# tmdt-buw/VQ-VAE-Transformer-Arc-Welding

Hardware: AMD Instinct MI355X
Metric: welding windows/sec (train) VQ-VAE+8-blk Transformer at 1/2/4/8 MI355X (higher is better)
Workload: dtype bf16; 1 GPU; VQ-VAE-Patch reconstruction train step (configs[1]); global_batch=1024, per_gpu_batch=1024, seq_len=200, codebook=512x64, hidden=512, n_resblocks=8, patch=25, parallelism=dp1, optimizer=RAdam(lr 1e-3), operands=bf16 (opt-in), fp32 accumulation and master weights

## Files before the change

### include/arcweld_amd.h

```cpp
#ifndef ARCWELD_AMD_H
#define ARCWELD_AMD_H

#include <stdint.h>

#ifdef __cplusplus
extern "C" {
#endif

enum { AW_OK = 0, AW_ERR_ARG = -1, AW_ERR_LAUNCH = -2 };
enum { AW_F32 = 0, AW_BF16 = 1 };
enum { AW_ACT_GELU_ERF = 0, AW_ACT_GELU_TANH = 1, AW_ACT_DERIV = 2 };

const char* aw_last_error(void);
int aw_version(void);

typedef struct {
  int M, N, K;
  int a_dtype;
  const void* A; int64_t lda; int a_trans;
  const void* B; int64_t ldb; int b_trans;
  int conv_cin, conv_seg, conv_dir, conv_operand;
  float alpha, beta;
  const float* bias;
  int act;
  const float* pre; int64_t ld_pre;
  const float* resid; int64_t ld_resid;
  float drop_p; uint64_t drop_seed;
  void* C; int64_t ldc; int c_dtype;
  void* C2; int64_t ldc2; int c2_mode; int c2_dtype;
  float drop2_p; uint64_t drop2_seed;
  double* colstats; int stats_mod;
  float* a_rowsum;
  int bias_mod;
  int accumulate, col_mod, col_mul, col_off;
  const uint64_t* seed_ptr;
  int pre_dtype;
  int store_policy;
  int resid_dtype;
} aw_gemm_args;
#define AW_STORE_NT 0
#define AW_STORE_WT 1

int aw_gemm(const aw_gemm_args* args, void* stream);
int64_t aw_gemm_workspace(const aw_gemm_args* args);
int aw_gemm_ws(const aw_gemm_args* args, float* ws, int64_t ws_elems, void* stream);
#define AW_GEMM_MAX_GROUPS 16
int aw_gemm_grouped(const aw_gemm_args* args, int n, void* stream);
int aw_gemm_set_tile(int bm);
int aw_gemm_describe(const aw_gemm_args* args, int* layout, uint32_t* epi, int* tile_rows, int* specialised,
                     int* ragged, int* splits);
int aw_gemm_set_wgrad_policy(int mode);
#define AW_WGRAD_BATCH_MAX 32
int64_t aw_wgrad_batch_workspace(const aw_gemm_args* args, int n);
int aw_wgrad_batch(const aw_gemm_args* args, int n, void* ws, int64_t ws_bytes, void* stream);
int aw_wgrad_set_spin_limit(int polls);

#define AW_RES_CHAIN_MAX 16
#define AW_RES_TAIL_MAX 8
typedef struct {
  int64_t N;
  int H, R;
  int taps, seg;
  const void* a0;
  const void* x0;
  const void* w1[AW_RES_CHAIN_MAX];
  const void* w2[AW_RES_CHAIN_MAX];
  const float* b1[AW_RES_CHAIN_MAX];
  const float* b2[AW_RES_CHAIN_MAX];
  void* dgelu_h[AW_RES_CHAIN_MAX];
  void* a1[AW_RES_CHAIN_MAX];
  void* dgelu_x[AW_RES_CHAIN_MAX];
  void* a[AW_RES_CHAIN_MAX];
  float drop_p;
  uint64_t drop_seed[AW_RES_CHAIN_MAX];
  const uint64_t* seed_ptr;
  int store_policy;
  uint64_t* drop_masks;
  int tail_k1;
  const void* tail_w[AW_RES_TAIL_MAX];
  const float* tail_bias;
  void* tail_y;
  double* tail_colstats;
} aw_res_chain_fwd_args;
typedef struct {
  int64_t N;
  int H, R;
  int taps, seg;
  const void* gx;
  const void* gxo;
  const void* x0;
  const void* w1t[AW_RES_CHAIN_MAX];
  const void* w2t[AW_RES_CHAIN_MAX];
  const void* dgelu_h[AW_RES_CHAIN_MAX];
  const void* dgelu_x[AW_RES_CHAIN_MAX];
  void* gh[AW_RES_CHAIN_MAX];
  void* gxo_out[AW_RES_CHAIN_MAX];
  float drop_p;
  int store_policy;
  const uint64_t* drop_masks;
} aw_res_chain_bwd_args;
int aw_res_chain_fwd(const aw_res_chain_fwd_args* args, void* stream);
int aw_res_chain_bwd(const aw_res_chain_bwd_args* args, void* stream);
int64_t aw_res_dropout_masks_bytes(int64_t N, int R);
int aw_res_dropout_masks(int64_t N, int R, float drop_p, const uint64_t* drop_seed, const uint64_t* seed_ptr,
                         void* masks, void* stream);
#define AW_RES_PACK_MAX 32
int aw_res_pack_weights(const void* const* src, void* const* fwd, void* const* bwd, int n, int taps, void* stream);
int aw_res_pack_weights_mixed(const void* const* src, void* const* fwd, void* const* bwd, const int* job_taps, int n,
                              int taps, void* stream);

int aw_vq_forward(const float* z, const float* E, int64_t N, int K, int D,
                  float* zq, int64_t* idx, float* counts, double* sqerr, void* stream);
int aw_vq_forward_ex(const float* z, const float* E, int64_t N, int K, int D, float* zq, int64_t* idx, float* counts,
                     double* sqerr, void* zq_copy, int copy_dtype, void* stream);
#define AW_VQ_COUNT_GROUPS_MAX 64
int aw_vq_forward_ex2(const float* z, const float* E, int64_t N, int K, int D, float* zq, int64_t* idx, float* counts,
                      int count_groups, double* sqerr, void* zq_copy, int copy_dtype, void* stream);
int aw_vq_finalize(const float* counts, const double* sqerr, int64_t N, int K, int D, float beta,
                   float* loss, float* perplexity, void* stream);
int aw_vq_finalize_ex(const float* counts, int count_groups, const double* sqerr, int64_t N, int K, int D, float beta,
                      float* loss, float* perplexity, void* stream);
int aw_vq_backward(const float* z, const float* E, const int64_t* idx, const float* g_zq, const float* g_loss,
                   int64_t N, int K, int D, float beta, float* dz, float* dE, void* stream);
int aw_vq_backward_ex(const float* z, const float* E, const int64_t* idx, const float* g_zq, const float* g_loss,
                      int64_t N, int K, int D, float beta, float* dz, float* dE, void* dz_copy, int copy_dtype,
                      void* stream);
int aw_vq_cluster_sums(const float* z, const int64_t* idx, int64_t N, int K, int D, float* sums, void* stream);
int aw_kmeans_update(float* means, const float* sums, const float* counts, int K, int D, float* avg, void* stream);
int aw_rvq_ema_update(float* embed, float* embed_avg, float* cluster_size, const float* counts, const float* sums,
                      const float* z, int64_t N, int K, int D, float decay, float eps, float threshold, uint64_t salt,
                      const uint64_t* seed_ptr, float* ws, void* stream);
int aw_rvq_residual(const float* r, const float* zq, int64_t n, float* out, int first, float* r_next, void* stream);
int aw_rvq_backward(const float* res, const float* q, const float* g_zq, const float* g_loss, int nq, int64_t N,
                    int D, float commitment, float* dz, void* stream);

int aw_vq_onehot(const int64_t* idx, int64_t N, int K, float* onehot, void* stream);
int aw_vq_gather(const float* E, const int64_t* idx, int64_t N, int D, float* out, void* stream);

int aw_patchify(const float* x, int64_t B, int L, int C, int P, void* patches, int64_t ldp, int dtype,
                void* stream);
int aw_weight_relayout(const float* W, int O, int I, int k, int tap, int mode, void* out, int64_t ldo,
                       int dtype, void* stream);
#define AW_RELAYOUT_MAX_JOBS 40
typedef struct {
  const float* W;
  void* out;
  int O, I, k, tap, mode;
  int64_t ldo;
} aw_relayout_job;
int aw_weight_relayout_batch(const aw_relayout_job* jobs, int n, int dtype, void* stream);
int aw_weight_grad_scatter(const float* g, int O, int I, int k, int tap, int mode, int64_t ldg, float* G,
                           void* stream);
int aw_cast(const float* in, int64_t n, void* out, int dtype, void* stream);

int aw_unpatch_head_fwd(const float* y, int64_t R, int H, int Q, const float* stats, const float* w2,
                        const float* b2, float* x_hat, void* stream);
int aw_bn_finalize(const double* colstats, int64_t n, int H, const float* gamma, const float* beta,
                   float* running_mean, float* running_var, int64_t* nbt, float eps, float momentum,
                   int training, float* stats, void* stream);
int aw_unpatch_head_bwd1(const float* y, int64_t R, int H, int Q, const float* stats, const float* w2,
                         const float* g_xhat, double* gsums, float* gw2, float* gb2, float* ggamma, float* gbeta,
                         void* stream);
int aw_unpatch_head_bwd2(const float* y, int64_t R, int H, int Q, const float* stats, const float* w2,
                         const float* g_xhat, const double* gsums, int training, void* g_y, int gy_dtype, float* db_y,
                         void* stream);
int aw_unpatch_head_fwd_ex(const void* y, int y_dtype, int64_t R, int H, int Q, const float* stats, const float* w2,
                           const float* b2, float* x_hat, void* stream);
int aw_unpatch_head_bwd1_ex(const void* y, int y_dtype, int64_t R, int H, int Q, const float* stats, const float* w2,
                            const float* g_xhat, double* gsums, float* gw2, float* gb2, float* ggamma, float* gbeta,
                            void* stream);
int aw_unpatch_head_bwd2_ex(const void* y, int y_dtype, int64_t R, int H, int Q, const float* stats, const float* w2,
                            const float* g_xhat, const double* gsums, int training, void* g_y, int gy_dtype,
                            float* db_y, void* stream);
int aw_unpatch_head_fwd_bwd1(const void* y, int y_dtype, int64_t R, int H, int Q, const float* stats, const float* w2,
                             const float* b2, const float* x, const float* gscale, float* x_hat, float* g_xhat,
                             double* sqerr, double* gsums, float* gw2, float* gb2, float* ggamma, float* gbeta,
                             void* stream);
int aw_bn_group_stats(const float* h, int64_t N, int H, int G, double* sums, void* stream);
int aw_bn_group_finalize(const double* sums, int64_t n, int H, int G, const float* gamma, const float* beta,
                         float* running_mean, float* running_var, int64_t* nbt, float eps, float momentum,
                         int training, float* stats, void* stream);
int aw_bn_apply(const float* h, int64_t N, int H, int G, const float* stats, int mode, const float* resid,
                float drop_p, uint64_t drop_seed, const uint64_t* seed_ptr, float* out, void* op, int op_dtype,
                void* stream);
int aw_bn_bwd_reduce(const float* h, int64_t N, int H, int G, const float* stats, const float* g_in, float drop_p,
                     uint64_t drop_seed, const uint64_t* seed_ptr, double* sums, void* stream);
int aw_bn_bwd_apply(const float* h, int64_t N, int H, int G, const float* stats, const float* g_in, float drop_p,
                    uint64_t drop_seed, const uint64_t* seed_ptr, const double* sums, int64_t n, int training,
                    void* dh, int dh_dtype, float* dgamma, float* dbeta, void* stream);
int aw_mse_fwd(const float* a, const float* b, int64_t n, double* sqerr, void* stream);
int aw_mse_bwd(const float* a, const float* b, int64_t n, const float* g, float* ga, void* stream);

int aw_scalar_add(const float* a, const float* b, float* out, void* stream);
int aw_mse_finalize(const double* sqerr, int64_t numel, float* out, void* stream);
int aw_mse_finalize_add(const double* sqerr, int64_t numel, const float* addend, float* out, float* sum, void* stream);

int aw_radam_step(float* param, float* grad, float* exp_avg, float* exp_avg_sq, const int64_t* seg_off,
                  const int64_t* seg_len, const float* seg_wd, const int* seg_active, int nseg, int64_t total, int64_t step,
                  float lr, float beta1, float beta2, float eps, const float* gscale, const int64_t* step_ptr,
                  int zero_grad, void* stream);
#define AW_OPS_PER_SEG 2
typedef struct {
  void* out;
  int O, I, k, tap, mode, dtype;
  int64_t ldo;
} aw_operand_desc;
int aw_radam_step_ops(float* param, float* grad, float* exp_avg, float* exp_avg_sq, const int64_t* seg_off,
                      const int64_t* seg_len, const float* seg_wd, const int* seg_active, int nseg, int64_t total,
                      int64_t step, float lr, float beta1, float beta2, float eps, const float* gscale,
                      const int64_t* step_ptr, const aw_operand_desc* ops, int zero_grad, void* stream);
int aw_counter_add(int64_t* counter, int64_t v, void* stream);
int aw_counter_add_snapshot(int64_t* counter, int64_t v, int64_t* snapshot, void* stream);
int aw_counter_add_snapshot_zero(int64_t* counter, int64_t v, int64_t* snapshot, double* zero, int64_t nzero,
                                 void* stream);
#define AW_NORM_WS 1024
int aw_grad_norm_clip(const float* grad, const int64_t* seg_off, const int64_t* seg_len, const int* seg_active,
                      int nseg, int64_t total, float max_norm, double* ws, float* out_norm, float* out_coef,
                      void* stream);
int aw_scale(float* x, int64_t n, const float* s, void* stream);

int aw_layernorm_fwd(const float* x, int64_t R, int D, const float* w, const float* b, float eps, void* y,
                     int y_dtype, float* mean, float* rstd, void* stream);
int aw_layernorm_bwd(const float* x, const float* dy, int64_t R, int D, const float* w, const float* mean,
                     const float* rstd, float* dx, int accumulate, float* dw, float* db, void* dx2, int dx2_dtype,
                     float drop_p, uint64_t drop_seed, const uint64_t* seed_ptr, void* stream);
int aw_class_head_fwd(const float* xf, int64_t B, int T, int D, const float* w1, const float* b1, const float* W2,
                      const float* b2, float* s, float* out, void* stream);
int aw_class_head_bwd(const float* xf, const float* s, const float* dout, int64_t B, int T, int D, const float* w1,
                      const float* W2, float* dxf, float* dw1, float* db1, float* dW2, float* db2, void* stream);
int aw_embed_fwd(const int64_t* ids, int64_t B, int T, int D, const float* wtok, const float* pe, float* x,
                 void* stream);
int aw_embed_ln_fwd(const int64_t* ids, int64_t B, int T, int D, const float* wtok, const float* pe, float* x,
                    const float* w, const float* b, float eps, void* y, int y_dtype, float* mean, float* rstd,
                    void* stream);
int aw_embed_bwd(const int64_t* ids, int64_t B, int T, int D, const float* dx, float* dwtok, void* stream);
int aw_embed_bwd_sorted(const int64_t* ids, int64_t B, int T, int D, int V, const float* dx, float* dwtok, int* work,
                        void* stream);
int aw_embed_sort(const int64_t* ids, int64_t R, int V, int* work, void* stream);
int aw_embed_bwd_segsum(const int* work, int V, int D, const float* dx, float* dwtok, void* stream);
int aw_attn_fwd(const void* qkv, int64_t B, int T, int n_head, int d, int dtype, void* y, float* lse,
                void* stream);
int aw_attn_bwd(const void* qkv, const void* y, const void* dy, const float* lse, int64_t B, int T, int n_head,
                int d, int dtype, void* dqkv, float* ws, void* stream);
int aw_attn_fwd_dropout(const void* qkv, int64_t B, int T, int n_head, int d, int dtype, void* y, float* lse,
                        float drop_p, uint64_t drop_seed, const uint64_t* seed_ptr, void* stream);
int aw_attn_bwd_dropout(const void* qkv, const void* y, const void* dy, const float* lse, int64_t B, int T,
                        int n_head, int d, int dtype, void* dqkv, float* ws, float drop_p, uint64_t drop_seed,
                        const uint64_t* seed_ptr, void* stream);
int aw_attn_decode(const void* qkv_new, int64_t B, int n_new, int pos0, int n_head, int d, int dtype,
                   void* kv_cache, int Tmax, void* y, void* stream);
int aw_ce_fwd(const float* logits, int64_t R, int V, int64_t ldl, const int64_t* y, int ignore_index,
              double* loss_sum, double* count, float* lse, void* stream);
int aw_ce_bwd(const float* logits, int64_t R, int V, int64_t ldl, const int64_t* y, int ignore_index,
              const float* lse, const double* count, const float* g, void* dlogits, int64_t ldd, int dtype,
              void* stream);
int aw_ce_finalize(const double* loss_sum, const double* count, float* out, void* stream);

int aw_gru_pack_weights(const float* w_hh, int H, int op_dtype, void* w_fwd, void* w_bwd, void* stream);
int aw_gru_step_fwd(int B, int H, int op_dtype, const void* h_prev_op, const float* h_prev, const void* w_fwd,
                    const float* gi, const float* b_hh, float* h, void* h_op, float* saved, void* stream);
int aw_gru_step_bwd(int B, int H, int op_dtype, const void* dgh_next_op, const float* dh_next,
                    const float* saved_next, const void* w_bwd, const float* dy, const float* saved,
                    const float* h_prev, float* dh, float* dgi, float* dgh, void* dgi_op, void* dgh_op, void* stream);
int aw_gru_bias_grad(const float* dg, int64_t rows, int H, float* db, void* stream);

#ifdef __cplusplus
}
#endif
#endif
```

### vq-vae-transformer-arc-welding_amd/arcweld/_native.py

```python
from __future__ import annotations

import ctypes
import os

import torch

PKG_DIR = os.path.dirname(os.path.dirname(os.path.abspath(__file__)))
LIB_PATH = os.environ.get("ARCWELD_LIB") or os.path.join(PKG_DIR, "lib", "libarcweld_amd.so")
HEADER = os.path.join(os.path.dirname(PKG_DIR), "include", "arcweld_amd.h")

AW_F32, AW_BF16 = 0, 1
AW_ACT_GELU_ERF, AW_ACT_GELU_TANH, AW_ACT_DERIV = 0, 1, 2
AW_STORE_NT, AW_STORE_WT = 0, 1

c_i64 = ctypes.c_int64
c_int = ctypes.c_int
c_f = ctypes.c_float
c_p = ctypes.c_void_p


class GemmArgs(ctypes.Structure):
    _fields_ = [
        ("M", c_int), ("N", c_int), ("K", c_int),
        ("a_dtype", c_int),
        ("A", c_p), ("lda", c_i64), ("a_trans", c_int),
        ("B", c_p), ("ldb", c_i64), ("b_trans", c_int),
        ("conv_cin", c_int), ("conv_seg", c_int), ("conv_dir", c_int), ("conv_operand", c_int),
        ("alpha", c_f), ("beta", c_f),
        ("bias", c_p),
        ("act", c_int),
        ("pre", c_p), ("ld_pre", c_i64),
        ("resid", c_p), ("ld_resid", c_i64),
        ("drop_p", c_f), ("drop_seed", ctypes.c_uint64),
        ("C", c_p), ("ldc", c_i64), ("c_dtype", c_int),
        ("C2", c_p), ("ldc2", c_i64), ("c2_mode", c_int), ("c2_dtype", c_int),
        ("drop2_p", c_f), ("drop2_seed", ctypes.c_uint64),
        ("colstats", c_p), ("stats_mod", c_int),
        ("a_rowsum", c_p),
        ("bias_mod", c_int),
        ("accumulate", c_int), ("col_mod", c_int), ("col_mul", c_int), ("col_off", c_int),
        ("seed_ptr", c_p),
        ("pre_dtype", c_int),
        ("store_policy", c_int),
        ("resid_dtype", c_int),
    ]


class RelayoutJob(ctypes.Structure):
    _fields_ = [("W", c_p), ("out", c_p), ("O", c_int), ("I", c_int), ("k", c_int), ("tap", c_int),
                ("mode", c_int), ("ldo", c_i64)]


class OperandDesc(ctypes.Structure):
    _fields_ = [("out", c_p), ("O", c_int), ("I", c_int), ("k", c_int), ("tap", c_int), ("mode", c_int),
                ("dtype", c_int), ("ldo", c_i64)]


OPS_PER_SEG = 2

RES_CHAIN_MAX = 16
RES_PACK_MAX = 32
RES_TAIL_MAX = 8
_E = RES_CHAIN_MAX


class ResChainFwdArgs(ctypes.Structure):
    _fields_ = [("N", c_i64), ("H", c_int), ("R", c_int), ("taps", c_int), ("seg", c_int), ("a0", c_p), ("x0", c_p),
                ("w1", c_p * _E), ("w2", c_p * _E), ("b1", c_p * _E), ("b2", c_p * _E),
                ("dgelu_h", c_p * _E), ("a1", c_p * _E), ("dgelu_x", c_p * _E), ("a", c_p * _E),
                ("drop_p", c_f), ("drop_seed", ctypes.c_uint64 * _E), ("seed_ptr", c_p), ("store_policy", c_int),
                ("drop_masks", c_p),
                ("tail_k1", c_int), ("tail_w", c_p * RES_TAIL_MAX), ("tail_bias", c_p), ("tail_y", c_p),
                ("tail_colstats", c_p)]


class ResChainBwdArgs(ctypes.Structure):
    _fields_ = [("N", c_i64), ("H", c_int), ("R", c_int), ("taps", c_int), ("seg", c_int), ("gx", c_p), ("gxo", c_p),
                ("x0", c_p), ("w1t", c_p * _E), ("w2t", c_p * _E), ("dgelu_h", c_p * _E), ("dgelu_x", c_p * _E),
                ("gh", c_p * _E), ("gxo_out", c_p * _E),
                ("drop_p", c_f), ("store_policy", c_int), ("drop_masks", c_p)]

SIGNATURES = {
    "aw_version": [],
    "aw_gemm": [ctypes.POINTER(GemmArgs), c_p],
    "aw_gemm_ws": [ctypes.POINTER(GemmArgs), c_p, c_i64, c_p],
    "aw_gemm_workspace": [ctypes.POINTER(GemmArgs)],
    "aw_gemm_grouped": [ctypes.POINTER(GemmArgs), c_int, c_p],
    "aw_gemm_set_tile": [c_int],
    "aw_gemm_describe": [ctypes.POINTER(GemmArgs), ctypes.POINTER(c_int), ctypes.POINTER(ctypes.c_uint32),
                         ctypes.POINTER(c_int), ctypes.POINTER(c_int), ctypes.POINTER(c_int), ctypes.POINTER(c_int)],
    "aw_gemm_set_wgrad_policy": [c_int],
    "aw_wgrad_batch_workspace": [ctypes.POINTER(GemmArgs), c_int],
    "aw_wgrad_batch": [ctypes.POINTER(GemmArgs), c_int, c_p, c_i64, c_p],
    "aw_wgrad_set_spin_limit": [c_int],
    "aw_res_chain_fwd": [ctypes.POINTER(ResChainFwdArgs), c_p],
    "aw_res_chain_bwd": [ctypes.POINTER(ResChainBwdArgs), c_p],
    "aw_res_pack_weights": [ctypes.POINTER(c_p), ctypes.POINTER(c_p), ctypes.POINTER(c_p), c_int, c_int, c_p],
    "aw_res_pack_weights_mixed": [ctypes.POINTER(c_p), ctypes.POINTER(c_p), ctypes.POINTER(c_p),
                                  ctypes.POINTER(c_int), c_int, c_int, c_p],
    "aw_res_dropout_masks_bytes": [c_i64, c_int],
    "aw_res_dropout_masks": [c_i64, c_int, c_f, ctypes.POINTER(ctypes.c_uint64), c_p, c_p, c_p],
    "aw_weight_relayout_batch": [ctypes.POINTER(RelayoutJob), c_int, c_int, c_p],
    "aw_vq_forward": [c_p, c_p, c_i64, c_int, c_int, c_p, c_p, c_p, c_p, c_p],
    "aw_vq_forward_ex": [c_p, c_p, c_i64, c_int, c_int, c_p, c_p, c_p, c_p, c_p, c_int, c_p],
    "aw_vq_finalize": [c_p, c_p, c_i64, c_int, c_int, c_f, c_p, c_p, c_p],
    "aw_vq_forward_ex2": [c_p, c_p, c_i64, c_int, c_int, c_p, c_p, c_p, c_int, c_p, c_p, c_int, c_p],
    "aw_vq_finalize_ex": [c_p, c_int, c_p, c_i64, c_int, c_int, c_f, c_p, c_p, c_p],
    "aw_vq_backward": [c_p, c_p, c_p, c_p, c_p, c_i64, c_int, c_int, c_f, c_p, c_p, c_p],
    "aw_vq_backward_ex": [c_p, c_p, c_p, c_p, c_p, c_i64, c_int, c_int, c_f, c_p, c_p, c_p, c_int, c_p],
    "aw_vq_onehot": [c_p, c_i64, c_int, c_p, c_p],
    "aw_vq_gather": [c_p, c_p, c_i64, c_int, c_p, c_p],
    "aw_patchify": [c_p, c_i64, c_int, c_int, c_int, c_p, c_i64, c_int, c_p],
    "aw_weight_relayout": [c_p, c_int, c_int, c_int, c_int, c_int, c_p, c_i64, c_int, c_p],
    "aw_weight_grad_scatter": [c_p, c_int, c_int, c_int, c_int, c_int, c_i64, c_p, c_p],
    "aw_cast": [c_p, c_i64, c_p, c_int, c_p],
    "aw_unpatch_head_fwd": [c_p, c_i64, c_int, c_int, c_p, c_p, c_p, c_p, c_p],
    "aw_bn_finalize": [c_p, c_i64, c_int, c_p, c_p, c_p, c_p, c_p, c_f, c_f, c_int, c_p, c_p],
    "aw_unpatch_head_bwd1": [c_p, c_i64, c_int, c_int, c_p, c_p, c_p, c_p, c_p, c_p, c_p, c_p, c_p],
    "aw_unpatch_head_bwd2": [c_p, c_i64, c_int, c_int, c_p, c_p, c_p, c_p, c_int, c_p, c_int, c_p, c_p],
    "aw_unpatch_head_fwd_ex": [c_p, c_int, c_i64, c_int, c_int, c_p, c_p, c_p, c_p, c_p],
    "aw_unpatch_head_bwd1_ex": [c_p, c_int, c_i64, c_int, c_int, c_p, c_p, c_p, c_p, c_p, c_p, c_p, c_p, c_p],
    "aw_unpatch_head_fwd_bwd1": [c_p, c_int, c_i64, c_int, c_int, c_p, c_p, c_p, c_p, c_p, c_p, c_p, c_p, c_p, c_p,
                                 c_p, c_p, c_p, c_p],
    "aw_unpatch_head_bwd2_ex": [c_p, c_int, c_i64, c_int, c_int, c_p, c_p, c_p, c_p, c_int, c_p, c_int, c_p, c_p],
    "aw_bn_group_stats": [c_p, c_i64, c_int, c_int, c_p, c_p],
    "aw_bn_group_finalize": [c_p, c_i64, c_int, c_int, c_p, c_p, c_p, c_p, c_p, c_f, c_f, c_int, c_p, c_p],
    "aw_bn_apply": [c_p, c_i64, c_int, c_int, c_p, c_int, c_p, c_f, ctypes.c_uint64, c_p, c_p, c_p, c_int, c_p],
    "aw_bn_bwd_reduce": [c_p, c_i64, c_int, c_int, c_p, c_p, c_f, ctypes.c_uint64, c_p, c_p, c_p],
    "aw_bn_bwd_apply": [c_p, c_i64, c_int, c_int, c_p, c_p, c_f, ctypes.c_uint64, c_p, c_p, c_i64, c_int, c_p, c_int,
                        c_p, c_p, c_p],
    "aw_mse_fwd": [c_p, c_p, c_i64, c_p, c_p],
    "aw_mse_bwd": [c_p, c_p, c_i64, c_p, c_p, c_p],
    "aw_scalar_add": [c_p, c_p, c_p, c_p],
    "aw_mse_finalize": [c_p, c_i64, c_p, c_p],
    "aw_mse_finalize_add": [c_p, c_i64, c_p, c_p, c_p, c_p],
    "aw_radam_step": [c_p, c_p, c_p, c_p, c_p, c_p, c_p, c_p, c_int, c_i64, c_i64, c_f, c_f, c_f, c_f, c_p, c_p,
                      c_int, c_p],
    "aw_radam_step_ops": [c_p, c_p, c_p, c_p, c_p, c_p, c_p, c_p, c_int, c_i64, c_i64, c_f, c_f, c_f, c_f, c_p, c_p,
                          c_p, c_int, c_p],
    "aw_counter_add": [c_p, c_i64, c_p],
    "aw_counter_add_snapshot": [c_p, c_i64, c_p, c_p],
    "aw_counter_add_snapshot_zero": [c_p, c_i64, c_p, c_p, c_i64, c_p],
    "aw_grad_norm_clip": [c_p, c_p, c_p, c_p, c_int, c_i64, c_f, c_p, c_p, c_p, c_p],
    "aw_scale": [c_p, c_i64, c_p, c_p],
    "aw_layernorm_fwd": [c_p, c_i64, c_int, c_p, c_p, c_f, c_p, c_int, c_p, c_p, c_p],
    "aw_layernorm_bwd": [c_p, c_p, c_i64, c_int, c_p, c_p, c_p, c_p, c_int, c_p, c_p, c_p, c_int, c_f,
                         ctypes.c_uint64, c_p, c_p],
    "aw_class_head_fwd": [c_p, c_i64, c_int, c_int, c_p, c_p, c_p, c_p, c_p, c_p, c_p],
    "aw_class_head_bwd": [c_p, c_p, c_p, c_i64, c_int, c_int, c_p, c_p, c_p, c_p, c_p, c_p, c_p, c_p],
    "aw_embed_fwd": [c_p, c_i64, c_int, c_int, c_p, c_p, c_p, c_p],
    "aw_embed_ln_fwd": [c_p, c_i64, c_int, c_int, c_p, c_p, c_p, c_p, c_p, c_f, c_p, c_int, c_p, c_p, c_p],
    "aw_embed_bwd": [c_p, c_i64, c_int, c_int, c_p, c_p, c_p],
    "aw_embed_bwd_sorted": [c_p, c_i64, c_int, c_int, c_int, c_p, c_p, c_p, c_p],
    "aw_embed_sort": [c_p, c_i64, c_int, c_p, c_p],
    "aw_embed_bwd_segsum": [c_p, c_int, c_int, c_p, c_p, c_p],
    "aw_attn_fwd": [c_p, c_i64, c_int, c_int, c_int, c_int, c_p, c_p, c_p],
    "aw_attn_bwd": [c_p, c_p, c_p, c_p, c_i64, c_int, c_int, c_int, c_int, c_p, c_p, c_p],
    "aw_attn_fwd_dropout": [c_p, c_i64, c_int, c_int, c_int, c_int, c_p, c_p, c_f, ctypes.c_uint64, c_p, c_p],
    "aw_attn_bwd_dropout": [c_p, c_p, c_p, c_p, c_i64, c_int, c_int, c_int, c_int, c_p, c_p, c_f, ctypes.c_uint64,
                            c_p, c_p],
    "aw_attn_decode": [c_p, c_i64, c_int, c_int, c_int, c_int, c_int, c_p, c_int, c_p, c_p],
    "aw_ce_fwd": [c_p, c_i64, c_int, c_i64, c_p, c_int, c_p, c_p, c_p, c_p],
    "aw_ce_bwd": [c_p, c_i64, c_int, c_i64, c_p, c_int, c_p, c_p, c_p, c_p, c_i64, c_int, c_p],
    "aw_ce_finalize": [c_p, c_p, c_p, c_p],
    "aw_vq_cluster_sums": [c_p, c_p, c_i64, c_int, c_int, c_p, c_p],
    "aw_kmeans_update": [c_p, c_p, c_p, c_int, c_int, c_p, c_p],
    "aw_rvq_ema_update": [c_p, c_p, c_p, c_p, c_p, c_p, c_i64, c_int, c_int, c_f, c_f, c_f, ctypes.c_uint64, c_p, c_p,
                          c_p],
    "aw_rvq_residual": [c_p, c_p, c_i64, c_p, c_int, c_p, c_p],
    "aw_rvq_backward": [c_p, c_p, c_p, c_p, c_int, c_i64, c_int, c_f, c_p, c_p],
    "aw_gru_pack_weights": [c_p, c_int, c_int, c_p, c_p, c_p],
    "aw_gru_step_fwd": [c_int, c_int, c_int, c_p, c_p, c_p, c_p, c_p, c_p, c_p, c_p, c_p],
    "aw_gru_bias_grad": [c_p, c_i64, c_int, c_p, c_p],
    "aw_gru_step_bwd": [c_int, c_int, c_int, c_p, c_p, c_p, c_p, c_p, c_p, c_p, c_p, c_p, c_p, c_p, c_p, c_p],
}

RET_I64 = {"aw_gemm_workspace", "aw_wgrad_batch_workspace", "aw_res_dropout_masks_bytes"}

_lib = None


class NativeError(RuntimeError):
    pass


def load(path: str = LIB_PATH):
    global _lib
    if _lib is not None:
        return _lib
    if not os.path.exists(path):
        raise NativeError(f"HIP library not built: {path} is missing (run `python -c 'import __graft_entry__ as g; "
                          f"g.build()'` or `make -C vq-vae-transformer-arc-welding_amd/csrc`)")
    lib = ctypes.CDLL(path, mode=ctypes.RTLD_GLOBAL)
    lib.aw_last_error.restype = ctypes.c_char_p
    lib.aw_last_error.argtypes = []
    for name, argtypes in SIGNATURES.items():
        fn = getattr(lib, name)
        fn.restype = c_i64 if name in RET_I64 else c_int
        fn.argtypes = argtypes
    _lib = lib
    return lib


def call(name: str, *args) -> None:
    lib = load()
    status = getattr(lib, name)(*args)
    if status != 0:
        raise NativeError(f"{name} failed ({status}): {lib.aw_last_error().decode(errors='replace')}")


def stream_ptr(stream=None) -> int:
    s = stream if stream is not None else torch.cuda.current_stream()
    return s.cuda_stream


def ptr(t):
    if t is None:
        return None
    if not t.is_cuda:
        raise NativeError("arcweld HIP kernels need device tensors (got a CPU tensor); there is no CPU fallback")
    return t.data_ptr()


def dtype_code(dt: torch.dtype) -> int:
    if dt == torch.float32:
        return AW_F32
    if dt == torch.bfloat16:
        return AW_BF16
    raise NativeError(f"unsupported operand dtype {dt}")
```

### vq-vae-transformer-arc-welding_amd/arcweld/kernels.py

```python
from __future__ import annotations

import contextvars
import ctypes

import torch

from . import _native as nat
from ._native import AW_ACT_DERIV, AW_ACT_GELU_ERF, AW_ACT_GELU_TANH, AW_BF16, AW_F32, GemmArgs, call, dtype_code, ptr, stream_ptr

__all__ = ["gemm", "AW_ACT_DERIV", "AW_ACT_GELU_ERF", "AW_ACT_GELU_TANH", "AW_BF16", "AW_F32"]


def _ld(t):
    if t is None:
        return 0
    if t.dim() == 1:
        return t.shape[0]
    if t.stride(-1) != 1:
        raise nat.NativeError("operand rows must be contiguous (stride(-1) == 1)")
    return t.stride(0)


_STORE_POLICY = contextvars.ContextVar("arcweld_store_policy", default=0)


class store_policy:

    def __init__(self, policy):
        self.policy = int(policy)

    def __enter__(self):
        self._tok = _STORE_POLICY.set(self.policy)

    def __exit__(self, *exc):
        _STORE_POLICY.reset(self._tok)
        return False

    def __call__(self, fn):
        import functools

        @functools.wraps(fn)
        def wrapped(*a, **k):
            with store_policy(self.policy):
                return fn(*a, **k)
        return wrapped


PROFILE = None


def _algorithmic_flops(M, N, Kd, conv, flops):
    if flops is not None:
        return float(flops)
    if conv is not None:
        seg = conv[1]
        return 2.0 * M * N * (Kd / 3.0) * (3.0 - 2.0 / seg)
    return 2.0 * M * N * Kd


def _gemm_args(A, B, M, N, K, *, a_trans=False, b_trans=False, conv=None, alpha=1.0, beta=0.0, bias=None,
               act=AW_ACT_GELU_ERF, pre=None, resid=None, drop=(0.0, 0), C=None, C2=None, c2_mode=0, drop2=(0.0, 0),
               colstats=None, stats_mod=0, a_rowsum=None, bias_mod=0, accumulate=False, col_map=(0, 1, 0),
               seed_ptr=None):
    if A.dtype != B.dtype:
        raise nat.NativeError(f"gemm operands must share a dtype ({A.dtype} vs {B.dtype})")
    a = GemmArgs()
    a.M, a.N, a.K = int(M), int(N), int(K)
    a.a_dtype = dtype_code(A.dtype)
    a.A, a.lda, a.a_trans = ptr(A), _ld(A), int(bool(a_trans))
    a.B, a.ldb, a.b_trans = ptr(B), _ld(B), int(bool(b_trans))
    if conv is not None:
        a.conv_cin, a.conv_seg, a.conv_dir, a.conv_operand = (int(v) for v in conv)
    a.alpha, a.beta = float(alpha), float(beta)
    a.bias = ptr(bias)
    a.act = int(act)
    a.store_policy = _STORE_POLICY.get()
    a.pre, a.ld_pre = ptr(pre), _ld(pre)
    if pre is not None:
        if pre.dtype not in (torch.float32, torch.bfloat16):
            raise nat.NativeError("pre must be float32 or bfloat16")
        a.pre_dtype = dtype_code(pre.dtype)
    a.resid, a.ld_resid = ptr(resid), _ld(resid)
    if resid is not None:
        if resid.dtype not in (torch.float32, torch.bfloat16):
            raise nat.NativeError("resid must be float32 or bfloat16")
        a.resid_dtype = dtype_code(resid.dtype)
    a.drop_p, a.drop_seed = float(drop[0]), int(drop[1]) & 0xFFFFFFFFFFFFFFFF
    if C is not None:
        a.C, a.ldc, a.c_dtype = ptr(C), _ld(C), dtype_code(C.dtype)
    if C2 is not None:
        a.C2, a.ldc2, a.c2_dtype = ptr(C2), _ld(C2), dtype_code(C2.dtype)
    a.c2_mode = int(c2_mode)
    a.drop2_p, a.drop2_seed = float(drop2[0]), int(drop2[1]) & 0xFFFFFFFFFFFFFFFF
    if colstats is not None:
        if colstats.dtype != torch.float64:
            raise nat.NativeError("colstats must be float64")
        a.colstats, a.stats_mod = ptr(colstats), int(stats_mod)
    a.a_rowsum = ptr(a_rowsum)
    a.bias_mod = int(bias_mod)
    a.accumulate = int(bool(accumulate))
    a.col_mod, a.col_mul, a.col_off = (int(v) for v in col_map)
    a.seed_ptr = ptr(seed_ptr)
    return a


def _timed(s, fn, flops, tag, name=None, nbytes=None):
    e0, e1 = torch.cuda.Event(enable_timing=True), torch.cuda.Event(enable_timing=True)
    e0.record(s)
    fn(s.cuda_stream)
    e1.record(s)
    PROFILE.append((e0, e1, flops, tag, name or tag, nbytes))


def _gemm_tag(A):
    return "gemm_bf16" if A.dtype == torch.bfloat16 else "gemm_f32"


def gemm(A, B, M, N, K, *, stream=None, flops=None, **kw):
    a = _gemm_args(A, B, M, N, K, **kw)
    lib = nat.load()
    wsn = lib.aw_gemm_workspace(ctypes.byref(a))
    ws = torch.empty(wsn, device=A.device, dtype=torch.float32) if wsn > 0 else None
    if PROFILE is None:
        call("aw_gemm_ws", ctypes.byref(a), ptr(ws), wsn, stream_ptr(stream))
        return kw.get("C")
    s = stream if stream is not None else torch.cuda.current_stream()
    _timed(s, lambda sp: call("aw_gemm_ws", ctypes.byref(a), ptr(ws), wsn, sp),
           _algorithmic_flops(M, N, K, kw.get("conv"), flops), _gemm_tag(A), "gemm_kernel")
    return kw.get("C")


MAX_GROUPS = 16


def gemm_grouped(problems, stream=None):
    for c0 in range(0, len(problems), MAX_GROUPS):
        chunk = problems[c0:c0 + MAX_GROUPS]
        arr = (GemmArgs * len(chunk))(*[_gemm_args(A, B, M, N, K, **kw) for (A, B, M, N, K, kw) in chunk])
        if PROFILE is None:
            call("aw_gemm_grouped", arr, len(chunk), stream_ptr(stream))
            continue
        s = stream if stream is not None else torch.cuda.current_stream()
        fl = sum(_algorithmic_flops(M, N, K, kw.get("conv"), None) for (_, _, M, N, K, kw) in chunk)
        c0_ = chunk[0]
        nm = "wgrad_conv3_kernel" if (c0_[5].get("conv") is not None and c0_[0].dtype == torch.bfloat16) \
            else "gemm_kernel (grouped)"
        _timed(s, lambda sp: call("aw_gemm_grouped", arr, len(chunk), sp), fl, _gemm_tag(chunk[0][0]), nm)


WGRAD_BATCH_MAX = 32


def wgrad_batch_ok(problems):
    import os
    mode = os.environ.get("ARCWELD_WGRAD_BATCH", "auto")
    if mode == "0" or not problems or len(problems) > WGRAD_BATCH_MAX:
        return False
    arr = (GemmArgs * len(problems))(*[_gemm_args(A, B, M, N, K, **kw) for (A, B, M, N, K, kw) in problems])
    if nat.load().aw_wgrad_batch_workspace(arr, len(problems)) <= 0:
        return False
    tiles = sum((M // 256) * (N // 256) for (_, _, M, N, _, _) in problems)
    return mode == "1" or tiles >= 128


def wgrad_batch(problems, stream=None):
    arr = (GemmArgs * len(problems))(*[_gemm_args(A, B, M, N, K, **kw) for (A, B, M, N, K, kw) in problems])
    lib = nat.load()
    wsb = lib.aw_wgrad_batch_workspace(arr, len(problems))
    if wsb < 0:
        raise nat.NativeError(f"aw_wgrad_batch: batch not eligible ({lib.aw_last_error().decode(errors='replace')})")
    ws = torch.empty((wsb + 3) // 4, device=problems[0][0].device, dtype=torch.float32)
    if PROFILE is None:
        call("aw_wgrad_batch", arr, len(problems), ptr(ws), wsb, stream_ptr(stream))
        return
    s = stream if stream is not None else torch.cuda.current_stream()
    fl = sum(_algorithmic_flops(M, N, K, None, None) for (_, _, M, N, K, _) in problems)
    _timed(s, lambda sp: call("aw_wgrad_batch", arr, len(problems), ptr(ws), wsb, sp), fl, _gemm_tag(problems[0][0]),
           "wgrad_tt_kernel")


def wgrad_issue(problems, stream=None):
    if not problems:
        return
    nch = (len(problems) + WGRAD_BATCH_MAX - 1) // WGRAD_BATCH_MAX
    per = (len(problems) + nch - 1) // nch
    chunks = [problems[i:i + per] for i in range(0, len(problems), per)]
    if all(wgrad_batch_ok(c) for c in chunks):
        for c in chunks:
            wgrad_batch(c, stream)
        return
    by_shape = {}
    for pb in problems:
        by_shape.setdefault((pb[2], pb[3]), []).append(pb)
    for grp in by_shape.values():
        gemm_grouped(grp, stream)


RES_CHAIN_MAX = nat.RES_CHAIN_MAX


def res_chain_ok(H, R, T, RT, taps=1, seg=16, which="ENC"):
    import os
    if os.environ.get(f"ARCWELD_{which}_CHAIN", "1") == "0":
        return False
    return (H == 512 and 1 <= R <= RES_CHAIN_MAX and T == torch.bfloat16 and RT == torch.bfloat16
            and (taps == 1 or (taps == 3 and seg == 16)))


def _chain_store_policy():
    import os
    return nat.AW_STORE_WT if os.environ.get("ARCWELD_CHAIN_STORE", "nt") == "wt" else nat.AW_STORE_NT


def _chk_rows(ts, N, H, who):
    for t in ts:
        if t is None:
            continue
        if t.dtype != torch.bfloat16 or t.dim() != 2 or tuple(t.shape) != (N, H) or not t.is_contiguous():
            raise nat.NativeError(f"{who}: activations must be contiguous ({N}, {H}) bfloat16 tensors")


def res_dropout_masks_empty(N, R, device):
    nb = nat.load().aw_res_dropout_masks_bytes(int(N), int(R))
    if nb <= 0:
        raise nat.NativeError("res_dropout_masks: bad N / R")
    return torch.empty(nb, device=device, dtype=torch.uint8)


def res_dropout_masks(N, drop, seed_ptr=None, stream=None):
    p, seeds = float(drop[0]), list(drop[1] or [])
    if p <= 0.0:
        return None
    R = len(seeds)
    out = res_dropout_masks_empty(N, R, torch.cuda.current_device() if seed_ptr is None else seed_ptr.device)
    sd = (ctypes.c_uint64 * R)(*[int(v) & 0xFFFFFFFFFFFFFFFF for v in seeds])
    call("aw_res_dropout_masks", int(N), R, p, sd, ptr(seed_ptr), ptr(out), stream_ptr(stream))
    return out


def _nbytes(ts):
    seen, n = set(), 0
    for t in ts:
        if t is not None and t.data_ptr() not in seen:
            seen.add(t.data_ptr())
            n += t.numel() * t.element_size()
    return n


def _chain_flops(R, N, H, taps, seg):
    if taps == 1:
        return 4.0 * R * N * H * H
    return 4.0 * R * N * H * H * (3 - 2.0 / seg)


def convt_tail_ok():
    import os
    return os.environ.get("ARCWELD_CONVT_TAIL", "1") != "0"


def res_chain_fwd(a0, x0, w1, w2, b1, b2, dh, a1, dx, a, drop=(0.0, None), seed_ptr=None, masks=None, taps=1, seg=16,
                  stream=None, tail=None):
    N, H = a0.shape
    R = len(w1)
    if not (1 <= R <= RES_CHAIN_MAX) or not all(len(v) == R for v in (w2, b1, b2, dh, a1, dx, a)):
        raise nat.NativeError("res_chain_fwd: need R (1..16) entries in every per-block list")
    _chk_rows([a0, x0] + list(dh) + list(a1) + list(dx) + list(a), N, H, "res_chain_fwd")
    g = nat.ResChainFwdArgs()
    g.N, g.H, g.R, g.taps, g.seg = N, H, R, int(taps), int(seg)
    g.a0, g.x0 = ptr(a0), ptr(x0)
    for r in range(R):
        g.w1[r], g.w2[r], g.b1[r], g.b2[r] = ptr(w1[r]), ptr(w2[r]), ptr(b1[r]), ptr(b2[r])
        g.dgelu_h[r], g.a1[r], g.dgelu_x[r], g.a[r] = ptr(dh[r]), ptr(a1[r]), ptr(dx[r]), ptr(a[r])
        g.drop_seed[r] = int(drop[1][r]) & 0xFFFFFFFFFFFFFFFF if drop[0] > 0 else 0
    g.drop_p = float(drop[0])
    g.seed_ptr = ptr(seed_ptr)
    g.store_policy = _chain_store_policy()
    g.drop_masks = ptr(masks)
    flops, extra = _chain_flops(R, N, H, taps, seg), []
    if tail is not None:
        wt, tb, Y, cst = tail
        k1 = len(wt)
        if taps != 3 or not (1 <= k1 <= nat.RES_TAIL_MAX):
            raise nat.NativeError(f"res_chain_fwd: the tail needs taps == 3 and 1..{nat.RES_TAIL_MAX} matrices")
        if Y.dtype != torch.bfloat16 or tuple(Y.shape) != (N, k1 * H) or not Y.is_contiguous():
            raise nat.NativeError(f"res_chain_fwd: tail Y must be a contiguous ({N}, {k1 * H}) bfloat16 tensor")
        if tb.dtype != torch.float32 or tb.numel() != H or not tb.is_contiguous():
            raise nat.NativeError("res_chain_fwd: tail bias must be (H,) float32")
        if cst is not None and (cst.dtype != torch.float64 or cst.numel() < 2 * H or not cst.is_contiguous()):
            raise nat.NativeError("res_chain_fwd: tail colstats must be (2 H,) float64")
        for w in wt:
            if w.dtype != torch.bfloat16 or w.numel() != H * H or not w.is_contiguous():
                raise nat.NativeError("res_chain_fwd: tail matrices must be packed (H, H) bfloat16 copies")
        g.tail_k1 = k1
        for j in range(k1):
            g.tail_w[j] = ptr(wt[j])
        g.tail_bias, g.tail_y, g.tail_colstats = ptr(tb), ptr(Y), ptr(cst)
        flops += 2.0 * N * k1 * H * H
        extra = [Y, tb] + list(wt)
    _maybe_timed(stream, "gemm_bf16", flops,
                 lambda sp: call("aw_res_chain_fwd", ctypes.byref(g), sp),
                 lambda: (f"res_chain_fwd_kernel<{int(taps)}>",
                          _nbytes([a0, x0, masks] + list(w1) + list(w2) + list(b1) + list(b2) + list(dh) + list(a1) +
                                  list(dx)[:-1] + list(a) + extra)))


def res_chain_bwd(gx, gxo, w1t, w2t, dh, x0, dx, gh, gxo_out, drop_p=0.0, masks=None, taps=1, seg=16, stream=None):
    N, H = gx.shape
    R = len(w1t)
    if not (1 <= R <= RES_CHAIN_MAX) or not all(len(v) == R for v in (w2t, dh, dx, gh, gxo_out)):
        raise nat.NativeError("res_chain_bwd: need R (1..16) entries in every per-block list")
    _chk_rows([gx, gxo, x0] + list(dh) + list(dx[1:]) + list(gh) + list(gxo_out), N, H, "res_chain_bwd")
    g = nat.ResChainBwdArgs()
    g.N, g.H, g.R, g.taps, g.seg = N, H, R, int(taps), int(seg)
    g.gx, g.gxo, g.x0 = ptr(gx), ptr(gxo), ptr(x0)
    for r in range(R):
        g.w1t[r], g.w2t[r], g.dgelu_h[r] = ptr(w1t[r]), ptr(w2t[r]), ptr(dh[r])
        g.dgelu_x[r] = ptr(dx[r]) if r > 0 else None
        g.gh[r], g.gxo_out[r] = ptr(gh[r]), ptr(gxo_out[r])
    g.drop_p = float(drop_p)
    g.store_policy = _chain_store_policy()
    g.drop_masks = ptr(masks)
    _maybe_timed(stream, "gemm_bf16", _chain_flops(R, N, H, taps, seg),
                 lambda sp: call("aw_res_chain_bwd", ctypes.byref(g), sp),
                 lambda: (f"res_chain_bwd_kernel<{int(taps)}>",
                          _nbytes([gx, gxo, x0, masks] + list(w1t) + list(w2t) + list(dh) + list(dx[1:]) + list(gh) +
                                  list(gxo_out))))


def res_pack_weights(src, fwd=None, bwd=None, taps=1, stream=None, job_taps=None):
    n = len(src)
    fwd = fwd if fwd is not None else [None] * n
    bwd = bwd if bwd is not None else [None] * n
    jt = [int(taps)] * n if job_taps is None else [int(v) for v in job_taps]
    if len(fwd) != n or len(bwd) != n or len(jt) != n:
        raise nat.NativeError("res_pack_weights: list lengths differ")
    for i in range(n):
        for t in (src[i], fwd[i], bwd[i]):
            if t is not None and (t.dtype != torch.bfloat16 or t.numel() != 512 * 512 * jt[i] or not t.is_contiguous()):
                raise nat.NativeError(f"res_pack_weights: need contiguous 512 x {512 * jt[i]} bfloat16 tensors")
    for c0 in range(0, n, nat.RES_PACK_MAX):
        sl = slice(c0, c0 + nat.RES_PACK_MAX)
        m = len(src[sl])
        arr = lambda ts: (ctypes.c_void_p * m)(*[ptr(t) for t in ts])
        if job_taps is None:
            call("aw_res_pack_weights", arr(src[sl]), arr(fwd[sl]), arr(bwd[sl]), m, int(taps), stream_ptr(stream))
        else:
            call("aw_res_pack_weights_mixed", arr(src[sl]), arr(fwd[sl]), arr(bwd[sl]), (ctypes.c_int * m)(*jt[sl]), m,
                 int(taps), stream_ptr(stream))


def vq_forward(z2d, E, zq, idx, counts, sqerr, stream=None, zq_copy=None, count_groups=1):
    N, D = z2d.shape
    Kc = E.shape[0]
    assert counts.numel() >= count_groups * Kc, "counts: count_groups x K floats"
    _maybe_timed(stream, "vq_fwd", 2.0 * N * Kc * D, lambda sp: call(
        "aw_vq_forward_ex2", ptr(z2d), ptr(E), N, Kc, D, ptr(zq), ptr(idx), ptr(counts), int(count_groups),
        ptr(sqerr), ptr(zq_copy), dtype_code(zq_copy.dtype) if zq_copy is not None else 0, sp),
        lambda: ("vq_fwd_pinned_kernel" if Kc <= 512 and D in (16, 32, 64) else "vq_fwd_kernel",
                 _nbytes([z2d, E, zq, idx, zq_copy]) + 4 * Kc * count_groups))


def vq_finalize(counts, sqerr, N, K, D, beta, loss, perplexity, stream=None, count_groups=1):
    call("aw_vq_finalize_ex", ptr(counts), int(count_groups), ptr(sqerr), N, K, D, float(beta), ptr(loss),
         ptr(perplexity), stream_ptr(stream))


def vq_backward(z2d, E, idx, g_zq, g_loss, beta, dz, dE, stream=None, dz_copy=None):
    N, D = z2d.shape
    if dz_copy is None:
        call("aw_vq_backward", ptr(z2d), ptr(E), ptr(idx), ptr(g_zq), ptr(g_loss), N, E.shape[0], D, float(beta),
             ptr(dz), ptr(dE), stream_ptr(stream))
    else:
        call("aw_vq_backward_ex", ptr(z2d), ptr(E), ptr(idx), ptr(g_zq), ptr(g_loss), N, E.shape[0], D, float(beta),
             ptr(dz), ptr(dE), ptr(dz_copy), dtype_code(dz_copy.dtype), stream_ptr(stream))


def vq_cluster_sums(z2d, idx, K, sums, stream=None):
    _dense(z2d, "vq_cluster_sums")
    call("aw_vq_cluster_sums", ptr(z2d), ptr(idx), z2d.shape[0], K, z2d.shape[1], ptr(sums), stream_ptr(stream))


def kmeans_update(means, sums, counts, avg=None, stream=None):
    call("aw_kmeans_update", ptr(means), ptr(sums), ptr(counts), means.shape[0], means.shape[1], ptr(avg),
         stream_ptr(stream))


def rvq_ema_update(embed, embed_avg, cluster_size, counts, sums, z2d, decay, eps, threshold, salt, seed_ptr, ws,
                   stream=None):
    K, D = embed.shape
    call("aw_rvq_ema_update", ptr(embed), ptr(embed_avg), ptr(cluster_size), ptr(counts), ptr(sums), ptr(z2d),
         z2d.shape[0], K, D, float(decay), float(eps), float(threshold), int(salt) & 0xFFFFFFFFFFFFFFFF,
         ptr(seed_ptr), ptr(ws), stream_ptr(stream))


def rvq_residual(r, zq, out, first, r_next=None, stream=None):
    call("aw_rvq_residual", ptr(r), ptr(zq), zq.numel(), ptr(out), int(bool(first)), ptr(r_next), stream_ptr(stream))


def rvq_backward(res, q, g_zq, g_loss, dz, commitment=1.0, stream=None):
    nq, N, D = res.shape
    call("aw_rvq_backward", ptr(res), ptr(q), ptr(g_zq), ptr(g_loss), nq, N, D, float(commitment), ptr(dz),
         stream_ptr(stream))


def vq_onehot(idx, K, out, stream=None):
    call("aw_vq_onehot", ptr(idx), idx.numel(), K, ptr(out), stream_ptr(stream))


def vq_gather(E, idx, out, stream=None):
    call("aw_vq_gather", ptr(E), ptr(idx), idx.numel(), E.shape[1], ptr(out), stream_ptr(stream))


def patchify(x, P, out, stream=None):
    B, L, C = x.shape
    call("aw_patchify", ptr(x), B, L, C, P, ptr(out), out.stride(0), dtype_code(out.dtype), stream_ptr(stream))


def weight_relayout(W, O, I, k, tap, mode, out, ldo=0, stream=None):
    _dense(W, "weight_relayout")
    call("aw_weight_relayout", ptr(W), O, I, k, tap, mode, ptr(out), ldo, dtype_code(out.dtype), stream_ptr(stream))


RELAYOUT_MAX_JOBS = 40


def _dense(W, who):
    if not W.is_contiguous():
        raise nat.NativeError(f"{who}: the source weight must be contiguous (got strides {tuple(W.stride())})")


def weight_relayout_batch(jobs, stream=None):
    by_dtype = {}
    for jb in jobs:
        by_dtype.setdefault(jb[6].dtype, []).append(jb)
    for dt, js in by_dtype.items():
        for c0 in range(0, len(js), RELAYOUT_MAX_JOBS):
            chunk = js[c0:c0 + RELAYOUT_MAX_JOBS]
            arr = (nat.RelayoutJob * len(chunk))()
            for r, jb in zip(arr, chunk):
                W, O, I, k, tap, mode, out = jb[:7]
                _dense(W, "weight_relayout_batch")
                r.W, r.out = ptr(W), ptr(out)
                r.O, r.I, r.k, r.tap, r.mode = int(O), int(I), int(k), int(tap), int(mode)
                r.ldo = int(jb[7]) if len(jb) > 7 else 0
            call("aw_weight_relayout_batch", arr, len(chunk), dtype_code(dt), stream_ptr(stream))


def weight_grad_scatter(g, O, I, k, tap, mode, G, stream=None):
    call("aw_weight_grad_scatter", ptr(g), O, I, k, tap, mode, g.stride(0), ptr(G), stream_ptr(stream))


def cast(x, out, stream=None):
    call("aw_cast", ptr(x), x.numel(), ptr(out), dtype_code(out.dtype), stream_ptr(stream))


def bn_finalize(colstats, n, H, gamma, beta, rm, rv, nbt, eps, momentum, training, stats, stream=None):
    call("aw_bn_finalize", ptr(colstats), n, H, ptr(gamma), ptr(beta), ptr(rm), ptr(rv), ptr(nbt), float(eps),
         float(momentum), int(training), ptr(stats), stream_ptr(stream))


def unpatch_head_fwd(y, Q, stats, w2, b2, x_hat, stream=None):
    R, H = y.shape
    call("aw_unpatch_head_fwd_ex", ptr(y), dtype_code(y.dtype), R, H, Q, ptr(stats), ptr(w2), ptr(b2), ptr(x_hat),
         stream_ptr(stream))


def unpatch_head_bwd1(y, Q, stats, w2, g_xhat, gsums, gw2, gb2, ggamma, gbeta, stream=None):
    R, H = y.shape
    call("aw_unpatch_head_bwd1_ex", ptr(y), dtype_code(y.dtype), R, H, Q, ptr(stats), ptr(w2), ptr(g_xhat), ptr(gsums),
         ptr(gw2), ptr(gb2), ptr(ggamma), ptr(gbeta), stream_ptr(stream))


def unpatch_head_bwd2(y, Q, stats, w2, g_xhat, gsums, training, g_y, db_y, stream=None):
    R, H = y.shape
    call("aw_unpatch_head_bwd2_ex", ptr(y), dtype_code(y.dtype), R, H, Q, ptr(stats), ptr(w2), ptr(g_xhat),
         ptr(gsums), int(training), ptr(g_y), dtype_code(g_y.dtype), ptr(db_y), stream_ptr(stream))


def unpatch_head_fwd_bwd1(y, Q, stats, w2, b2, x, gscale, x_hat, g_xhat, sqerr, gsums, gw2, gb2, ggamma, gbeta,
                          stream=None):
    R, H = y.shape
    for nm, t in (("x", x), ("x_hat", x_hat), ("g_xhat", g_xhat)):
        if t.dtype != torch.float32 or not t.is_contiguous() or t.numel() != R * 5:
            raise nat.NativeError(f"unpatch_head_fwd_bwd1: {nm} must be a contiguous float32 tensor of R*5 = {R * 5} "
                                  f"elements (got {tuple(t.shape)} {t.dtype}, contiguous={t.is_contiguous()})")
    call("aw_unpatch_head_fwd_bwd1", ptr(y), dtype_code(y.dtype), R, H, Q, ptr(stats), ptr(w2), ptr(b2), ptr(x),
         ptr(gscale), ptr(x_hat), ptr(g_xhat), ptr(sqerr), ptr(gsums), ptr(gw2), ptr(gb2), ptr(ggamma), ptr(gbeta),
         stream_ptr(stream))


def head_bf16_ok(H):
    return 64 <= H <= 2048 and H & (H - 1) == 0


def mse_fwd(a, b, sqerr, stream=None):
    call("aw_mse_fwd", ptr(a), ptr(b), a.numel(), ptr(sqerr), stream_ptr(stream))


def mse_bwd(a, b, g, ga, stream=None):
    call("aw_mse_bwd", ptr(a), ptr(b), a.numel(), ptr(g), ptr(ga), stream_ptr(stream))


def scalar_add(a, b, out, stream=None):
    call("aw_scalar_add", ptr(a), ptr(b), ptr(out), stream_ptr(stream))


def mse_finalize(sqerr, numel, out, stream=None):
    call("aw_mse_finalize", ptr(sqerr), int(numel), ptr(out), stream_ptr(stream))


def mse_finalize_add(sqerr, numel, addend, out, total, stream=None):
    call("aw_mse_finalize_add", ptr(sqerr), int(numel), ptr(addend), ptr(out), ptr(total), stream_ptr(stream))


def radam_step(param, grad, m, v, seg_off, seg_len, seg_wd, seg_active, nseg, total, step, lr, beta1, beta2, eps,
               gscale=None, stream=None, step_ptr=None, ops=None, zero_grad=False):
    args = (ptr(param), ptr(grad), ptr(m), ptr(v), ptr(seg_off), ptr(seg_len), ptr(seg_wd), ptr(seg_active), int(nseg),
            int(total), int(step), float(lr), float(beta1), float(beta2), float(eps), ptr(gscale), ptr(step_ptr))
    if ops is None:
        call("aw_radam_step", *args, int(bool(zero_grad)), stream_ptr(stream))
    else:
        call("aw_radam_step_ops", *args, ptr(ops), int(bool(zero_grad)), stream_ptr(stream))


def counter_add_snapshot(counter, snapshot, v=1, stream=None, zero=None):
    if zero is None:
        call("aw_counter_add_snapshot", ptr(counter), int(v), ptr(snapshot), stream_ptr(stream))
        return
    if zero.dtype != torch.float64 or not zero.is_contiguous():
        raise nat.NativeError("counter_add_snapshot: zero must be a contiguous float64 tensor")
    call("aw_counter_add_snapshot_zero", ptr(counter), int(v), ptr(snapshot), ptr(zero), zero.numel(),
         stream_ptr(stream))


def counter_add(counter, v=1, stream=None):
    call("aw_counter_add", ptr(counter), int(v), stream_ptr(stream))


NORM_WS = 1024


def grad_norm_clip(grad, seg_off, seg_len, seg_active, nseg, max_norm, ws, out_norm, out_coef, stream=None):
    if ws.numel() < NORM_WS or ws.dtype != torch.float64:
        raise nat.NativeError(f"grad_norm_clip: ws must hold {NORM_WS} float64")
    call("aw_grad_norm_clip", ptr(grad), ptr(seg_off), ptr(seg_len), ptr(seg_active), int(nseg), grad.numel(),
         float(max_norm), ptr(ws), ptr(out_norm), ptr(out_coef), stream_ptr(stream))


def scale_(x, s, stream=None):
    call("aw_scale", ptr(x), x.numel(), ptr(s), stream_ptr(stream))


def layernorm_fwd(x, w, b, eps, y, mean, rstd, stream=None):
    R, D = x.shape
    call("aw_layernorm_fwd", ptr(x), R, D, ptr(w), ptr(b), float(eps), ptr(y), dtype_code(y.dtype), ptr(mean),
         ptr(rstd), stream_ptr(stream))


def layernorm_bwd(x, dy, w, mean, rstd, dx, accumulate, dw, db, dx2=None, drop=(0.0, 0), stream=None,
                  seed_ptr=None):
    R, D = x.shape
    call("aw_layernorm_bwd", ptr(x), ptr(dy), R, D, ptr(w), ptr(mean), ptr(rstd), ptr(dx), int(accumulate), ptr(dw),
         ptr(db), ptr(dx2), dtype_code(dx2.dtype) if dx2 is not None else AW_F32, float(drop[0]),
         int(drop[1]) & 0xFFFFFFFFFFFFFFFF, ptr(seed_ptr), stream_ptr(stream))


def class_head_fwd(xf, B, T, w1, b1, W2, b2, s, out, stream=None):
    call("aw_class_head_fwd", ptr(xf), B, T, xf.shape[-1], ptr(w1), ptr(b1), ptr(W2), ptr(b2), ptr(s), ptr(out),
         stream_ptr(stream))


def class_head_bwd(xf, s, dout, B, T, w1, W2, dxf, dw1, db1, dW2, db2, stream=None):
    call("aw_class_head_bwd", ptr(xf), ptr(s), ptr(dout), B, T, xf.shape[-1], ptr(w1), ptr(W2), ptr(dxf), ptr(dw1),
         ptr(db1), ptr(dW2), ptr(db2), stream_ptr(stream))


def embed_fwd(ids, wtok, pe, x, stream=None):
    B, T = ids.shape
    call("aw_embed_fwd", ptr(ids), B, T, wtok.shape[1], ptr(wtok), ptr(pe), ptr(x), stream_ptr(stream))


def embed_ln_fwd(ids, wtok, pe, x, w, b, eps, y, mean, rstd, stream=None):
    B, T = ids.shape
    call("aw_embed_ln_fwd", ptr(ids), B, T, wtok.shape[1], ptr(wtok), ptr(pe), ptr(x), ptr(w), ptr(b), float(eps),
         ptr(y), dtype_code(y.dtype), ptr(mean), ptr(rstd), stream_ptr(stream))


def embed_bwd(ids, dx, dwtok, stream=None, sort=True):
    B, T = ids.shape
    if not sort:
        call("aw_embed_bwd", ptr(ids), B, T, dwtok.shape[1], ptr(dx), ptr(dwtok), stream_ptr(stream))
        return
    V = dwtok.shape[0]
    work = torch.empty(V + 1 + B * T, device=dx.device, dtype=torch.int32)
    call("aw_embed_bwd_sorted", ptr(ids), B, T, dwtok.shape[1], V, ptr(dx), ptr(dwtok), ptr(work),
         stream_ptr(stream))


EMBED_SORT_MAX_V = 15360


def embed_sort(ids, V, work, stream=None):
    call("aw_embed_sort", ptr(ids), ids.numel(), V, ptr(work), stream_ptr(stream))


def embed_bwd_segsum(work, dx, dwtok, stream=None):
    call("aw_embed_bwd_segsum", ptr(work), dwtok.shape[0], dwtok.shape[1], ptr(dx), ptr(dwtok), stream_ptr(stream))


def attn_flops(B, T, n_head, d):
    return 4.0 * B * n_head * (T * (T + 1) / 2) * (d // n_head)


def _maybe_timed(stream, tag, flops, fn, info=None):
    if PROFILE is None:
        fn(stream_ptr(stream))
        return
    s = stream if stream is not None else torch.cuda.current_stream()
    _timed(s, fn, flops, tag, *(info() if info is not None else ()))


def attn_fwd(qkv, B, T, n_head, d, y, lse, drop=(0.0, 0), seed_ptr=None, stream=None):
    if drop[0] > 0:
        _maybe_timed(stream, "attn_fwd", attn_flops(B, T, n_head, d), lambda sp: call(
            "aw_attn_fwd_dropout", ptr(qkv), B, T, n_head, d, dtype_code(qkv.dtype), ptr(y), ptr(lse),
            float(drop[0]), int(drop[1]) & 0xFFFFFFFFFFFFFFFF, ptr(seed_ptr), sp))
        return
    _maybe_timed(stream, "attn_fwd", attn_flops(B, T, n_head, d), lambda sp: call(
        "aw_attn_fwd", ptr(qkv), B, T, n_head, d, dtype_code(qkv.dtype), ptr(y), ptr(lse), sp))


def attn_bwd(qkv, y, dy, lse, B, T, n_head, d, dqkv, ws, drop=(0.0, 0), seed_ptr=None, stream=None):
    fl = 2.0 * attn_flops(B, T, n_head, d)
    if drop[0] > 0:
        _maybe_timed(stream, "attn_bwd", fl, lambda sp: call(
            "aw_attn_bwd_dropout", ptr(qkv), ptr(y), ptr(dy), ptr(lse), B, T, n_head, d, dtype_code(qkv.dtype),
            ptr(dqkv), ptr(ws), float(drop[0]), int(drop[1]) & 0xFFFFFFFFFFFFFFFF, ptr(seed_ptr), sp))
        return
    _maybe_timed(stream, "attn_bwd", fl, lambda sp: call(
        "aw_attn_bwd", ptr(qkv), ptr(y), ptr(dy), ptr(lse), B, T, n_head, d, dtype_code(qkv.dtype), ptr(dqkv),
        ptr(ws), sp))


def bn_group_stats(h, G, sums, stream=None):
    N, H = h.shape
    call("aw_bn_group_stats", ptr(h), N, H, int(G), ptr(sums), stream_ptr(stream))


def bn_group_finalize(sums, n, H, G, bn, training, stats, stream=None):
    mom = bn.momentum if bn.momentum is not None else 0.1
    call("aw_bn_group_finalize", ptr(sums) if training else None, int(n), int(H), int(G), ptr(bn.weight),
         ptr(bn.bias), ptr(bn.running_mean), ptr(bn.running_var), ptr(bn.num_batches_tracked) if training else None,
         float(bn.eps), float(mom), int(bool(training)), ptr(stats), stream_ptr(stream))


def bn_apply(h, G, stats, mode, out, op=None, resid=None, drop=(0.0, 0), seed_ptr=None, stream=None):
    N, H = h.shape
    call("aw_bn_apply", ptr(h), N, H, int(G), ptr(stats), int(mode), ptr(resid), float(drop[0]), int(drop[1]),
         ptr(seed_ptr), ptr(out), ptr(op), dtype_code(op.dtype) if op is not None else AW_F32, stream_ptr(stream))


def bn_bwd_reduce(h, G, stats, g_in, sums, drop=(0.0, 0), seed_ptr=None, stream=None):
    N, H = h.shape
    call("aw_bn_bwd_reduce", ptr(h), N, H, int(G), ptr(stats), ptr(g_in), float(drop[0]), int(drop[1]),
         ptr(seed_ptr), ptr(sums), stream_ptr(stream))


def bn_bwd_apply(h, G, stats, g_in, sums, n, training, dh, dgamma=None, dbeta=None, drop=(0.0, 0), seed_ptr=None,
                 stream=None):
    N, H = h.shape
    call("aw_bn_bwd_apply", ptr(h), N, H, int(G), ptr(stats), ptr(g_in), float(drop[0]), int(drop[1]),
         ptr(seed_ptr), ptr(sums), int(n), int(bool(training)), ptr(dh), dtype_code(dh.dtype), ptr(dgamma),
         ptr(dbeta), stream_ptr(stream))


def attn_decode(qkv_new, B, n_new, pos0, n_head, d, kv_cache, y, stream=None):
    if kv_cache.dtype != qkv_new.dtype or y.dtype != qkv_new.dtype or kv_cache.shape[-1] != 2 * d:
        raise nat.NativeError("attn_decode: qkv, cache and y share a dtype; cache rows are [K | V] (2d)")
    call("aw_attn_decode", ptr(qkv_new), B, n_new, pos0, n_head, d, dtype_code(qkv_new.dtype), ptr(kv_cache),
         kv_cache.shape[1], ptr(y), stream_ptr(stream))


def ce_fwd(logits, V, y, ignore_index, loss_sum, count, lse, stream=None):
    R = y.numel()
    call("aw_ce_fwd", ptr(logits), R, V, logits.stride(0), ptr(y), int(ignore_index), ptr(loss_sum), ptr(count),
         ptr(lse), stream_ptr(stream))


def ce_bwd(logits, V, y, ignore_index, lse, count, g, dlogits, stream=None):
    R = y.numel()
    call("aw_ce_bwd", ptr(logits), R, V, logits.stride(0), ptr(y), int(ignore_index), ptr(lse), ptr(count), ptr(g),
         ptr(dlogits), dlogits.stride(0), dtype_code(dlogits.dtype), stream_ptr(stream))


def ce_finalize(loss_sum, count, out, stream=None):
    call("aw_ce_finalize", ptr(loss_sum), ptr(count), ptr(out), stream_ptr(stream))


def gru_padded(H):
    return (int(H) + 31) // 32 * 32


def _chk_gru(name, t, shape, dtype):
    if t is None:
        return
    if t.dtype != dtype or tuple(t.shape) != tuple(shape) or not t.is_contiguous():
        raise nat.NativeError(f"gru: {name} must be a contiguous {dtype} tensor of shape {tuple(shape)}, got "
                              f"{t.dtype} {tuple(t.shape)}")


def gru_pack_weights(w_hh, H, w_fwd=None, w_bwd=None, stream=None):
    Hp = gru_padded(H)
    T = (w_fwd if w_fwd is not None else w_bwd).dtype
    _chk_gru("w_hh", w_hh, (3 * H, H), torch.float32)
    _chk_gru("w_fwd", w_fwd, (3, Hp, Hp), T)
    _chk_gru("w_bwd", w_bwd, (Hp, 3 * Hp), T)
    call("aw_gru_pack_weights", ptr(w_hh), int(H), dtype_code(T), ptr(w_fwd), ptr(w_bwd), stream_ptr(stream))


def gru_step_fwd(H, T, gi, b_hh, h, saved, w_fwd=None, h_prev_op=None, h_prev=None, h_op=None, stream=None):
    B, Hp = gi.shape[0], gru_padded(H)
    _chk_gru("gi", gi, (B, 3 * Hp), torch.float32)
    _chk_gru("b_hh", b_hh, (3 * H,), torch.float32)
    _chk_gru("h", h, (B, Hp), torch.float32)
    _chk_gru("saved", saved, (B, 4 * Hp), torch.float32)
    _chk_gru("h_prev_op", h_prev_op, (B, Hp), T)
    _chk_gru("h_prev", h_prev, (B, Hp), torch.float32)
    _chk_gru("h_op", h_op, (B, Hp), torch.bfloat16)
    _chk_gru("w_fwd", w_fwd, (3, Hp, Hp), T)
    call("aw_gru_step_fwd", B, int(H), dtype_code(T), ptr(h_prev_op), ptr(h_prev), ptr(w_fwd), ptr(gi), ptr(b_hh),
         ptr(h), ptr(h_op), ptr(saved), stream_ptr(stream))


def gru_step_bwd(H, T, saved, dh, dgi, dgh, w_bwd=None, dgh_next_op=None, dh_next=None, saved_next=None, dy=None,
                 h_prev=None, dgi_op=None, dgh_op=None, stream=None):
    B, Hp = saved.shape[0], gru_padded(H)
    f32 = torch.float32
    _chk_gru("saved", saved, (B, 4 * Hp), f32)
    _chk_gru("saved_next", saved_next, (B, 4 * Hp), f32)
    for name, t in (("dh", dh), ("dh_next", dh_next), ("dy", dy), ("h_prev", h_prev)):
        _chk_gru(name, t, (B, Hp), f32)
    for name, t in (("dgi", dgi), ("dgh", dgh)):
        _chk_gru(name, t, (B, 3 * Hp), f32)
    for name, t in (("dgi_op", dgi_op), ("dgh_op", dgh_op)):
        _chk_gru(name, t, (B, 3 * Hp), torch.bfloat16)
    _chk_gru("dgh_next_op", dgh_next_op, (B, 3 * Hp), T)
    _chk_gru("w_bwd", w_bwd, (Hp, 3 * Hp), T)
    call("aw_gru_step_bwd", B, int(H), dtype_code(T), ptr(dgh_next_op), ptr(dh_next), ptr(saved_next), ptr(w_bwd),
         ptr(dy), ptr(saved), ptr(h_prev), ptr(dh), ptr(dgi), ptr(dgh), ptr(dgi_op), ptr(dgh_op), stream_ptr(stream))


def gru_bias_grad(dg, H, db, stream=None):
    rows = dg.shape[0]
    _chk_gru("dg", dg, (rows, 3 * gru_padded(H)), torch.float32)
    _chk_gru("db", db, (3 * H,), torch.float32)
    call("aw_gru_bias_grad", ptr(dg), rows, int(H), ptr(db), stream_ptr(stream))
```

### vq-vae-transformer-arc-welding_amd/arcweld/resstack.py

```python
from __future__ import annotations

import torch

from . import kernels as K

F32 = torch.float32


def _centre_job(w, out):
    O, I = w.shape[0], w.shape[1]
    c = w[:, :, 1]
    if w.is_contiguous():
        return (w, O, I, 3, 1, 0, out)
    if not c.is_contiguous():
        raise ValueError("encoder conv weight: unsupported layout")
    return (c, O, I, 1, 0, 0, out)


def _centre_grad(g):
    O, I = g.shape[0], g.shape[1]
    if g.is_contiguous():
        return g.view(O, 3 * I), (0, 3, 1)
    c = g[:, :, 1]
    if not c.is_contiguous():
        raise ValueError("encoder conv gradient: unsupported layout")
    return c, (0, 1, 0)


def _conv3_job(w, mode, out):
    from .operands import OperandJob
    return OperandJob("", w, w.shape[0], w.shape[1], 3, 0, mode, out).relayout_job()


def _conv3_grad(g):
    O, I = g.shape[0], g.shape[1]
    if g.is_contiguous():
        return g.view(O, 3 * I), (I, 3, 0)
    st = g.permute(0, 2, 1)
    if not st.is_contiguous():
        raise ValueError("decoder conv gradient: unsupported layout")
    return st.reshape(O, 3 * I), (0, 1, 0)


class Geometry:

    def __init__(self, taps, H, S):
        self.taps, self.H, self.S, self.Kd = taps, H, S, taps * H
        conv = lambda d, operand: dict(conv=(H, S, d, operand)) if taps == 3 else {}
        self.fwd, self.dgrad, self.wgrad = conv(1, 0), conv(-1, 0), conv(1, 1)
        self.G = S if taps == 1 else 1
        self.grad_target = _centre_grad if taps == 1 else _conv3_grad

    def fwd_job(self, w, out):
        return _centre_job(w, out) if self.taps == 1 else _conv3_job(w, 1, out)

    def dgrad_job(self, w, out):
        return _conv3_job(w, 2, out)

    def wgrad_problem(self, A, B, gw, gb):
        Cw, cm = self.grad_target(gw)
        return (A, B, self.H, self.Kd, A.shape[0], dict(a_trans=True, b_trans=True, C=Cw, accumulate=True, col_map=cm,
                                                        a_rowsum=gb, **self.wgrad))


class Saved:

    def __init__(self, geo, route, T, p_drop, seeds, ctr, training, x0, a0):
        self.geo = geo
        self.route, self.T, self.p_drop, self.seeds, self.ctr, self.training = route, T, p_drop, seeds, ctr, training
        self.xs, self.a0s, self.hs, self.a1s, self.bs, self.ws = [x0], [a0], [], [], [], []
        self.masks = self.pk_bwd = None


def _bn_stats(h, G, bn, training):
    N, H = h.shape
    sums = None
    if training and N // G <= 1:
        raise ValueError(f"Expected more than 1 value per channel when training, got input size "
                         f"torch.Size([{N // G}, {H}])")
    if training:
        sums = torch.zeros(2, G, H, device=h.device, dtype=torch.float64)
        K.bn_group_stats(h, G, sums)
    st = torch.empty(4, G, H, device=h.device)
    K.bn_group_finalize(sums, N // G, H, G, bn, training, st)
    return st


def _bn_block_fwd(geo, a0, x, w1, w2, b1, b2, bns, training, p_drop, seed, ctr, T, last):
    N, H = x.shape
    G = geo.G
    bn1, bn2 = bns
    e = lambda *s, dt=F32: torch.empty(*s, device=x.device, dtype=dt)
    h1 = e(N, H)
    K.gemm(a0, w1, N, H, geo.Kd, bias=b1, C=h1, **geo.fwd)
    st1 = _bn_stats(h1, G, bn1, training)
    hn1, a1 = e(N, H), e(N, H, dt=T)
    K.bn_apply(h1, G, st1, 0, hn1, op=a1)
    h2 = e(N, H)
    K.gemm(a1, w2, N, H, geo.Kd, bias=b2, C=h2, **geo.fwd)
    st2 = _bn_stats(h2, G, bn2, training)
    y, an = e(N, H), e(N, H, dt=T)
    K.bn_apply(h2, G, st2, 2 if last else 1, y, op=an, resid=x, drop=(p_drop, seed), seed_ptr=ctr)
    return y, an, dict(h1=h1, hn1=hn1, a1=a1, h2=h2, st1=st1, st2=st2)


def _bn_block_bwd(sv, r, gy, w1d, w2d, grads, bns, slot, wgrads, need_copy):
    N, H = gy.shape
    geo = sv.geo
    G, T, training = geo.G, sv.T, sv.training
    bs, drop = sv.bs[r], dict(drop=(sv.p_drop, sv.seeds[r]), seed_ptr=sv.ctr)
    bn1, bn2 = bns
    dev = gy.device
    e = lambda *s, dt=F32: torch.empty(*s, device=dev, dtype=dt)
    n = N // G
    sums2 = torch.zeros(2, G, H, device=dev, dtype=torch.float64)
    K.bn_bwd_reduce(bs["h2"], G, bs["st2"], gy, sums2, **drop)
    dh2 = e(N, H, dt=T)
    K.bn_bwd_apply(bs["h2"], G, bs["st2"], gy, sums2, n, training, dh2, slot(bn2.weight), slot(bn2.bias), **drop)
    t1 = e(N, H)
    K.gemm(dh2, w2d, N, H, geo.Kd, b_trans=True, pre=bs["hn1"], C=t1, **geo.dgrad)
    wgrads.append(geo.wgrad_problem(dh2, bs["a1"], *grads(r, 1)))
    sums1 = torch.zeros(2, G, H, device=dev, dtype=torch.float64)
    K.bn_bwd_reduce(bs["h1"], G, bs["st1"], t1, sums1)
    dh1 = e(N, H, dt=T)
    K.bn_bwd_apply(bs["h1"], G, bs["st1"], t1, sums1, n, training, dh1, slot(bn1.weight), slot(bn1.bias))
    gx = e(N, H)
    gxo = e(N, H, dt=T) if need_copy else None
    K.gemm(dh1, w1d, N, H, geo.Kd, b_trans=True, pre=sv.xs[r], resid=gy, C=gx, C2=gxo, c2_mode=2 if need_copy else 0,
           **geo.dgrad)
    wgrads.append(geo.wgrad_problem(dh1, sv.a0s[r], *grads(r, 0)))
    return gx, gxo


def _chain_fwd(sv, weights, biases, RT, save, tail=None):
    geo = sv.geo
    R, H, taps, T = len(biases), geo.H, geo.taps, sv.T
    x0, a0 = sv.xs[0], sv.a0s[0]
    N, dev = a0.shape[0], a0.device
    e = lambda dt: torch.empty(N, H, device=dev, dtype=dt)
    sv.hs = [e(T) if save else None for _ in range(R)]
    sv.a1s = [e(T) if save else None for _ in range(R)]
    sv.xs += [e(RT) if save and r < R - 1 else None for r in range(R)]
    sv.a0s += [e(T) for _ in range(R)]
    wsrc = [w for r in range(R) for w in weights[r]]
    pk = [torch.empty(H, geo.Kd, device=dev, dtype=T) for _ in wsrc]
    ktail = None
    if tail is not None:
        Wt, tb, Y, cst = tail
        k1 = Wt.shape[0] // H
        tsrc = [Wt[j * H:(j + 1) * H] for j in range(k1)]
        tpk = [torch.empty(H, H, device=dev, dtype=T) for _ in tsrc]
        K.res_pack_weights(wsrc + tsrc, pk + tpk, None, taps=taps, job_taps=[taps] * len(wsrc) + [1] * k1)
        ktail = (tpk, tb, Y, cst)
    else:
        K.res_pack_weights(wsrc, pk, None, taps=taps)
    if save:
        sv.pk_bwd = wsrc
        if sv.p_drop > 0 and R > 1:
            sv.masks = K.res_dropout_masks_empty(N, R, dev)
    K.res_chain_fwd(a0, x0, pk[0::2], pk[1::2], [b1 for b1, _ in biases], [b2 for _, b2 in biases], sv.hs, sv.a1s,
                    sv.xs[1:], sv.a0s[1:], drop=(sv.p_drop, sv.seeds), seed_ptr=sv.ctr, masks=sv.masks, taps=taps,
                    seg=geo.S, tail=ktail)


def _chain_bwd(sv, gx, gxo, grads):
    N, H = gx.shape
    geo = sv.geo
    R, taps, dev, T = len(sv.hs), geo.taps, gx.device, gxo.dtype
    gh = [torch.empty(N, H, device=dev, dtype=T) for _ in range(R)]
    go = [torch.empty(N, H, device=dev, dtype=T) for _ in range(R)]
    pk_bwd = [torch.empty(H, geo.Kd, device=dev, dtype=T) for _ in sv.pk_bwd]
    K.res_pack_weights(sv.pk_bwd, None, pk_bwd, taps=taps)
    K.res_chain_bwd(gx, gxo, pk_bwd[0::2], pk_bwd[1::2], sv.hs, sv.xs[0], [None] + list(sv.xs[1:R]), gh, go,
                    drop_p=sv.p_drop, masks=sv.masks, taps=taps, seg=geo.S)
    sv.pk_bwd = sv.masks = None
    wgrads = []
    for r in reversed(range(R)):
        gin = gxo if r == R - 1 else go[r + 1]
        wgrads.append(geo.wgrad_problem(gin, sv.a1s[r], *grads(r, 1)))
        wgrads.append(geo.wgrad_problem(gh[r], sv.a0s[r], *grads(r, 0)))
    return go[0], wgrads


def forward(geo, x0, a0, weights, biases, bns=None, *, T, RT, p_drop=0.0, seeds=None, ctr=None, training=False,
            chain=False, last_operand_only=True, in_place=False, save=True, tail=None):
    R, H, Kd = len(biases), geo.H, geo.Kd
    N, dev = a0.shape[0], a0.device
    seeds = [0] * R if seeds is None else seeds
    route = "bn" if bns is not None else "chain" if chain else "conv"
    sv = Saved(geo, route, T, p_drop, seeds, ctr, training, x0, a0)
    e = lambda dt: torch.empty(N, H, device=dev, dtype=dt)
    if tail is not None and (route != "chain" or geo.taps != 3):
        raise ValueError("resstack.forward: the ConvT tail runs only inside the decoder chain")
    if route == "chain":
        _chain_fwd(sv, weights, biases, RT, save, tail)
        return sv.xs[R], sv.a0s[R], sv
    x, a, h, a1 = x0, a0, None, None
    for r in range(R):
        (w1, w2), (b1, b2) = weights[r], biases[r]
        last = last_operand_only and r == R - 1
        if route == "bn":
            xn, an, bs = _bn_block_fwd(geo, a, x, w1, w2, b1, b2, bns[r], training, p_drop, seeds[r], ctr, T, last)
        else:
            if h is None or not in_place:
                h, a1 = e(T), e(T)
            K.gemm(a, w1, N, H, Kd, bias=b1, C=h, C2=a1, c2_mode=1, **geo.fwd)
            xn = None if last else x if in_place else e(RT)
            an = a if in_place else e(T)
            out = dict(C=an) if last else dict(C=xn, C2=an, c2_mode=1)
            K.gemm(a1, w2, N, H, Kd, bias=b2, drop=(p_drop, seeds[r]), seed_ptr=ctr, resid=x, **out, **geo.fwd)
            bs = None
        if save:
            sv.xs.append(xn)
            sv.a0s.append(an)
            sv.hs.append(h)
            sv.a1s.append(a1)
            sv.bs.append(bs)
            sv.ws.append((w1, w2))
        x, a = xn, an
    return x, a, sv


def backward(sv, gy, go, dweights, grads, bns=None, slot=None, r0_copy=True):
    if sv.route == "chain":
        gxo, wgrads = _chain_bwd(sv, gy, go, grads)
        return gxo, gxo, wgrads
    N, H = gy.shape
    geo, RT, T, p = sv.geo, gy.dtype, sv.T, sv.p_drop
    e = lambda dt: torch.empty(N, H, device=gy.device, dtype=dt)
    wgrads = []
    for r in reversed(range(len(sv.hs))):
        W1d, W2d = dweights[r]
        if sv.route == "bn":
            gy, go = _bn_block_bwd(sv, r, gy, W1d, W2d, grads, bns[r], slot, wgrads, r0_copy and r == 0)
            continue
        gh = e(T)
        K.gemm(go, W2d, N, H, geo.Kd, b_trans=True, pre=sv.hs[r], C=gh, **geo.dgrad)
        wgrads.append(geo.wgrad_problem(go, sv.a1s[r], *grads(r, 1)))
        gyn = e(RT)
        gon = e(T) if r > 0 or r0_copy else None
        K.gemm(gh, W1d, N, H, geo.Kd, b_trans=True, pre=sv.xs[r], resid=gy, C=gyn, C2=gon,
               c2_mode=3 if r > 0 else 2 if r0_copy else 0, drop2=(p, sv.seeds[r - 1] if r > 0 else 0),
               seed_ptr=sv.ctr, **geo.dgrad)
        wgrads.append(geo.wgrad_problem(gh, sv.a0s[r], *grads(r, 0)))
        gy, go = gyn, gon
    return gy, go, wgrads
```

### vq-vae-transformer-arc-welding_amd/arcweld/vqvae.py

```python
from __future__ import annotations

import os
import weakref

import torch

from . import _native as nat
from . import kernels as K
from . import operands
from . import resstack
from .precision import operand_dtype

F32 = torch.float32


def _mix(seed: int, salt: int) -> int:
    z = (seed * 0x9E3779B97F4A7C15 + salt * 0xBF58476D1CE4E5B9 + 0x94D049BB133111EB) & 0xFFFFFFFFFFFFFFFF
    z ^= z >> 31
    z = (z * 0xD6E8FEB86659FD93) & 0xFFFFFFFFFFFFFFFF
    return z ^ (z >> 32)


def rng_snapshot(m, dev, p_drop, zero=None):
    if p_drop <= 0.0:
        if zero is not None:
            zero.zero_()
        return None
    ctr = getattr(m, "_rng_counter", None)
    if ctr is None or ctr.device != dev:
        ctr = torch.zeros(1, dtype=torch.int64, device=dev)
        m._rng_counter = ctr
    snap = torch.empty(1, dtype=torch.int64, device=dev)
    K.counter_add_snapshot(ctr, snap, zero=zero)
    return snap


VQ_COUNT_GROUPS = 8


def accumulators(m, dev, K, H, zero=True):
    key = (dev, K, H)
    st = m.__dict__.get("_acc_block")
    if st is None or st[0] != key:
        st = (key, torch.empty(2 + 4 * H + (VQ_COUNT_GROUPS * K + 1) // 2, dtype=torch.float64, device=dev))
        m.__dict__["_acc_block"] = st
    buf = st[1]
    if zero:
        buf.zero_()
    return dict(block=buf, vq_sq=buf[0:1], mse_sq=buf[1:2], colstats=buf[2:2 + 2 * H], head_gsums=buf[2 + 2 * H:2 + 4 * H],
                counts=buf[2 + 4 * H:].view(torch.float32)[:VQ_COUNT_GROUPS * K])


def resid_dtype(m, T):
    if T == F32 or m.batch_norm or os.environ.get("ARCWELD_RESID_F32", "0") == "1":
        return F32
    return T


class VQVAEShapes:
    def __init__(self, m, B):
        self.B = B
        self.H, self.D, self.K = m.hidden_dim, m.embedding_dim, m.num_embeddings
        self.R = m.n_resblocks
        self.P, self.L, self.C = m.patch_size, m.seq_len, m.input_dim
        self.S = self.L * self.C // self.P
        self.N = B * self.S
        self.k1 = m.reverse_patch_embed.k1
        self.Q = self.S * self.k1
        self.ldp = (self.P + 7) // 8 * 8


def _params(m):
    enc = [(blk.block[1], blk.block[4]) for blk in m.encoder[0].shared_conv]
    dec = [(blk.block[1], blk.block[4]) for blk in m.decoder[1].shared_conv]
    enc_bn = [(blk.block[2], blk.block[5]) for blk in m.encoder[0].shared_conv] if m.batch_norm else None
    dec_bn = [(blk.block[2], blk.block[5]) for blk in m.decoder[1].shared_conv] if m.batch_norm else None
    rp = m.reverse_patch_embed.proj
    E = None if getattr(m, "use_improved_vq", False) else m.vector_quantization.embedding.weight
    return dict(pe=m.patch_embed.proj, enc=enc, sep=m.encoder[1].shared_conv, E=E,
                dec0=m.decoder[0], dec=dec, t1=rp[0], bn=rp[1], t2=rp[3], enc_bn=enc_bn, dec_bn=dec_bn)


class Saved:
    pass


def _operand_jobs(m, T):
    from .operands import OperandJob as J
    sh = VQVAEShapes(m, 1)
    H, D, R, P, k1 = sh.H, sh.D, sh.R, sh.P, sh.k1
    pr = _params(m)
    dev = pr["pe"].weight.device
    e = lambda *s: torch.empty(*s, device=dev, dtype=T)
    jobs = [J("Wp", pr["pe"].weight, H, 1, P, 0, 4, torch.zeros(H, sh.ldp, device=dev, dtype=T),
              sh.ldp)]
    centre = lambda w: resstack._centre_job(w, None)[:6]
    for r, (c1, c2) in enumerate(pr["enc"]):
        for nm, c in (("1", c1), ("2", c2)):
            jobs.append(J(f"enc{r}_{nm}", c.weight, H, H, 1, 0, 0, e(H, H), derive=centre))
    jobs.append(J("Ws", pr["sep"].weight, D, H, 1, 0, 0, e(D, H)))
    jobs.append(J("Wd0", pr["dec0"].weight, H, D, 1, 0, 0, e(H, D)))
    for r, (c1, c2) in enumerate(pr["dec"]):
        for nm, c in (("1", c1), ("2", c2)):
            jobs.append(J(f"dec{r}_{nm}", c.weight, H, H, 3, 0, 1, e(H, 3 * H)))
            jobs.append(J(f"dgw{r}_{nm}", c.weight, H, H, 3, 0, 2, e(3 * H, H)))
    jobs.append(J("Wt1", pr["t1"].weight, H, H, k1, 0, 3, e(k1 * H, H)))
    return jobs


def operand_set(m, T=None):
    T = operand_dtype(T)
    return operands.peek(m, ("vqvae", T), lambda: _operand_jobs(m, T))


@K.store_policy(nat.AW_STORE_WT)
def forward(m, x, training: bool, need_backward: bool, dtype=None, seed: int = 0, head=True):
    T = operand_dtype(dtype)
    if x.dtype != F32 or x.dim() != 3:
        raise ValueError("VQVAEPatch expects float32 windows of shape (B, seq_len, input_dim)")
    x = x.contiguous()
    sh = VQVAEShapes(m, x.shape[0])
    H, D, N, S, R, P, k1 = sh.H, sh.D, sh.N, sh.S, sh.R, sh.P, sh.k1
    if x.shape[1] != sh.L or x.shape[2] != sh.C:
        raise ValueError(f"expected windows (B, {sh.L}, {sh.C}), got {tuple(x.shape)}")
    pr = _params(m)
    dev = x.device
    p_drop = float(m.dropout_p) if training else 0.0
    e = lambda *s, dt=F32: torch.empty(*s, device=dev, dtype=dt)
    sv = Saved()
    sv.sh, sv.T, sv.p_drop, sv.training = sh, T, p_drop, training
    RT = sv.RT = resid_dtype(m, T)
    acc = accumulators(m, dev, sh.K, H, zero=False)
    sv.ctr = rng_snapshot(m, dev, p_drop, zero=acc["block"])
    sv.acc = acc
    owner = m.__dict__.get("_acc_owner")
    owned = owner is not None and owner() is not None
    sv.head_gsums = acc["head_gsums"] if not owned else torch.zeros(2 * H, device=dev, dtype=torch.float64)
    if need_backward and not owned:
        m.__dict__["_acc_owner"] = weakref.ref(sv)

    ops = operands.get(m, ("vqvae", T), lambda: _operand_jobs(m, T))
    Wp, Ws, Wd0, Wt1 = ops["Wp"], ops["Ws"], ops["Wd0"], ops["Wt1"]
    enc_w = [(ops[f"enc{r}_1"], ops[f"enc{r}_2"]) for r in range(R)]
    dec_w = [(ops[f"dec{r}_1"], ops[f"dec{r}_2"]) for r in range(R)]
    sv.ops = ops

    patches = e(N, sh.ldp, dt=T)
    K.patchify(x, P, patches)
    x0, a0 = e(N, H, dt=RT), e(N, H, dt=T)
    K.gemm(patches, Wp, N, H, sh.ldp, bias=pr["pe"].bias, C=x0, C2=a0, c2_mode=1, flops=2 * N * H * P)

    stack = dict(T=T, RT=RT, p_drop=p_drop, ctr=sv.ctr, training=training, save=need_backward)
    _, xR_T, sv.enc = resstack.forward(resstack.Geometry(1, H, S), x0, a0, enc_w, _biases(pr["enc"]), pr["enc_bn"],
                                       seeds=[_mix(seed, 100 + r) for r in range(R)],
                                       chain=K.res_chain_ok(H, R, T, RT), **stack)
    if R == 0:
        xR_T = _operand(x0, T)

    z = e(N, D)
    K.gemm(xR_T, Ws, N, D, H, bias=pr["sep"].bias, C=z)

    Kc = sh.K
    if pr["E"] is None:
        rvq = m.vector_quantization.vq
        zq, idx2, losses, sv.rvq = rvq.quantize_rows(z, training, save=need_backward)
        idx = idx2[:, 0] if rvq.num_quantizers == 1 else idx2
        emb_loss = losses.view(()) if rvq.num_quantizers == 1 else losses.sum()
        perplexity = None
    else:
        zq = e(N, D)
        idx = e(N, dt=torch.int64)
        counts, sq = acc["counts"], acc["vq_sq"]
        zq_T = None if T == F32 else e(N, D, dt=T)
        K.vq_forward(z, pr["E"], zq, idx, counts, sq, zq_copy=zq_T, count_groups=VQ_COUNT_GROUPS)
        emb_loss, perplexity = e(()), e(())
        K.vq_finalize(counts, sq, N, Kc, D, m.vector_quantization.beta, emb_loss, perplexity,
                      count_groups=VQ_COUNT_GROUPS)
    if pr["E"] is None or T == F32:
        zq_T = zq if T == F32 else _cast(zq, T)

    y0, ya0 = e(N, H, dt=RT), e(N, H, dt=T)
    K.gemm(zq_T, Wd0, N, H, D, bias=pr["dec0"].bias, C=y0, C2=ya0, c2_mode=1)
    bf_y = T != F32 and K.head_bf16_ok(H) and os.environ.get("ARCWELD_HEAD_BF16", "1") == "1"
    Y = e(N, k1 * H, dt=T if bf_y else F32)
    colstats = acc["colstats"] if training else None
    dec_chain = K.res_chain_ok(H, R, T, RT, 3, S, "DEC") and pr["dec_bn"] is None
    convt_tail = dec_chain and bf_y and k1 <= nat.RES_TAIL_MAX and K.convt_tail_ok()
    _, yR_T, sv.dec = resstack.forward(resstack.Geometry(3, H, S), y0, ya0, dec_w, _biases(pr["dec"]), pr["dec_bn"],
                                       seeds=[_mix(seed, 200 + r) for r in range(R)], chain=dec_chain,
                                       tail=(Wt1, pr["t1"].bias, Y, colstats) if convt_tail else None, **stack)
    if R == 0:
        yR_T = _operand(y0, T)

    bn = pr["bn"]
    if not convt_tail:
        K.gemm(yR_T, Wt1, N, k1 * H, H, bias=pr["t1"].bias, bias_mod=H, C=Y, colstats=colstats, stats_mod=H)
    stats = e(4 * H)
    K.bn_finalize(colstats, N * k1, H, bn.weight, bn.bias, bn.running_mean, bn.running_var,
                  bn.num_batches_tracked if training else None, bn.eps,
                  bn.momentum if bn.momentum is not None else 0.1, training, stats)
    x_hat = e(sh.B, sh.L, sh.C)
    Y2 = Y.view(N * k1, H)
    sv.head_fused = not head and need_backward and fused_head_ok(H)
    if not sv.head_fused:
        K.unpatch_head_fwd(Y2, sh.Q, stats, pr["t2"].weight.view(H, 5), pr["t2"].bias, x_hat)

    if not need_backward:
        return emb_loss, x_hat, perplexity, idx, None
    sv.patches, sv.xR_T, sv.z, sv.idx, sv.zq_T, sv.yR_T = patches, xR_T, z, idx, zq_T, yR_T
    sv.Y2, sv.stats = Y2, stats
    sv.Ws, sv.Wd0, sv.Wt1 = Ws, Wd0, Wt1
    return emb_loss, x_hat, perplexity, idx, sv


def fused_head_ok(H):
    return H == 512


def head_train(m, sv, x, gscale, x_hat, sqerr, slot):
    sh, H = sv.sh, sv.sh.H
    pr = _params(m)
    bn = pr["bn"]
    g_xhat = torch.empty_like(x_hat)
    K.unpatch_head_fwd_bwd1(sv.Y2, sh.Q, sv.stats, pr["t2"].weight.view(H, 5), pr["t2"].bias, x, gscale, x_hat,
                            g_xhat, sqerr, sv.head_gsums, slot(pr["t2"].weight).view(H, 5), slot(pr["t2"].bias),
                            slot(bn.weight), slot(bn.bias))
    sv.head_pass1_done = True
    return g_xhat


@torch.no_grad()
def encode(m, x, dtype=F32):
    T = F32 if dtype is None else operand_dtype(dtype)
    if x.dtype != F32 or x.dim() != 3:
        raise ValueError("expected float32 windows of shape (W, seq_len, input_dim)")
    x = x.contiguous()
    sh = VQVAEShapes(m, x.shape[0])
    H, D, N, R, P = sh.H, sh.D, sh.N, sh.R, sh.P
    if x.shape[1] != sh.L or x.shape[2] != sh.C:
        raise ValueError(f"expected windows (W, {sh.L}, {sh.C}), got {tuple(x.shape)}")
    pr = _params(m)
    e = lambda *s, dt=F32: torch.empty(*s, device=x.device, dtype=dt)
    Wp = e(H, sh.ldp, dt=T)
    K.weight_relayout(pr["pe"].weight, H, 1, P, 0, 4, Wp, ldo=sh.ldp)
    patches = e(N, sh.ldp, dt=T)
    K.patchify(x, P, patches)
    xr, a = e(N, H), e(N, H, dt=T)
    K.gemm(patches, Wp, N, H, sh.ldp, bias=pr["pe"].bias, C=xr, C2=a, c2_mode=1, flops=2 * N * H * P)
    ew = [(e(H, H, dt=T), e(H, H, dt=T)) for _ in range(R)]
    Ws = e(D, H, dt=T)
    geo = resstack.Geometry(1, H, sh.S)
    K.weight_relayout_batch([geo.fwd_job(c.weight, w) for cs, ws in zip(pr["enc"], ew) for c, w in zip(cs, ws)]
                            + [(pr["sep"].weight, D, H, 1, 0, 0, Ws)])
    _, xR_T, _ = resstack.forward(geo, xr, a, ew, _biases(pr["enc"]), pr["enc_bn"], T=T, RT=F32, training=m.training,
                                  in_place=True, save=False)
    if R == 0:
        xR_T = _operand(xr, T)
    z = e(N, D)
    K.gemm(xR_T, Ws, N, D, H, bias=pr["sep"].bias, C=z)
    if pr["E"] is None:
        rvq = m.vector_quantization.vq
        if rvq.num_quantizers != 1:
            raise ValueError("tokenization needs a single quantizer (ResidualVQ num_quantizers == 1)")
        _, idx2, _, _ = rvq.quantize_rows(z, False)
        return idx2[:, 0].contiguous(), z
    zq, idx = e(N, D), e(N, dt=torch.int64)
    counts = torch.zeros(sh.K, device=x.device)
    sq = torch.zeros(1, device=x.device, dtype=torch.float64)
    K.vq_forward(z, pr["E"], zq, idx, counts, sq)
    return idx, z


def _cast(t, T):
    out = torch.empty(t.shape, device=t.device, dtype=T)
    K.cast(t, out)
    return out


def _operand(x, T):
    return x if x.dtype == T else _cast(x, T)


def _biases(convs):
    return [(c1.bias, c2.bias) for c1, c2 in convs]


def _grads(convs, slot):
    return lambda r, i: (slot(convs[r][i].weight), slot(convs[r][i].bias))


@K.store_policy(nat.AW_STORE_WT)
def backward(m, sv, g_emb, g_xhat, slot, mid_hook=None):
    sh, T, p_drop = sv.sh, sv.T, sv.p_drop
    H, D, N, S, R, P, k1 = sh.H, sh.D, sh.N, sh.S, sh.R, sh.P, sh.k1
    pr = _params(m)
    dev = g_xhat.device
    e = lambda *s, dt=F32: torch.empty(*s, device=dev, dtype=dt)
    g_xhat = g_xhat.contiguous()
    bn = pr["bn"]

    gsums = sv.head_gsums
    owner = m.__dict__.get("_acc_owner")
    if owner is not None and owner() is sv:
        m.__dict__["_acc_owner"] = None
    if not getattr(sv, "head_pass1_done", False):
        K.unpatch_head_bwd1(sv.Y2, sh.Q, sv.stats, pr["t2"].weight.view(H, 5), g_xhat, gsums,
                            slot(pr["t2"].weight).view(H, 5), slot(pr["t2"].bias), slot(bn.weight), slot(bn.bias))
    gY = e(N * k1, H, dt=T)
    K.unpatch_head_bwd2(sv.Y2, sh.Q, sv.stats, pr["t2"].weight.view(H, 5), g_xhat, gsums, sv.training, gY,
                        slot(pr["t1"].bias))
    gY2 = gY.view(N, k1 * H)
    K.gemm(sv.yR_T, gY2, H, k1 * H, N, a_trans=True, b_trans=True, C=slot(pr["t1"].weight).view(H, H * k1),
           accumulate=True, col_map=(H, k1, 0))
    RT = sv.RT
    gy, go = e(N, H, dt=RT), e(N, H, dt=T)
    bnm = m.batch_norm and R > 0
    K.gemm(gY2, sv.Wt1, N, H, k1 * H, b_trans=True, C=gy, C2=None if bnm else go, c2_mode=0 if bnm else
           (3 if R > 0 else 2), drop2=(p_drop, sv.dec.seeds[-1] if R > 0 else 0), seed_ptr=sv.ctr)

    dgw = [(sv.ops[f"dgw{r}_1"], sv.ops[f"dgw{r}_2"]) for r in range(R)]
    gy, go, wgrads = resstack.backward(sv.dec, gy, go, dgw, _grads(pr["dec"], slot), pr["dec_bn"], slot)
    K.gemm_grouped(wgrads)

    K.gemm(go, sv.zq_T, H, D, N, a_trans=True, b_trans=True, C=slot(pr["dec0"].weight).view(H, D), accumulate=True,
           a_rowsum=slot(pr["dec0"].bias))
    gzq = e(N, D)
    K.gemm(go, sv.Wd0, N, D, H, b_trans=True, C=gzq)

    dz = e(N, D)
    dz_T = dz if T == F32 else None
    if pr["E"] is None:
        res, qs = sv.rvq
        nq = res.shape[0]
        K.rvq_backward(res, qs, gzq, g_emb if nq == 1 else g_emb.expand(nq).contiguous(), dz)
    else:
        dz_T = dz if T == F32 else e(N, D, dt=T)
        K.vq_backward(sv.z, pr["E"], sv.idx, gzq, g_emb, m.vector_quantization.beta, dz, slot(pr["E"]),
                      dz_copy=None if T == F32 else dz_T)
    if mid_hook is not None:
        with K.store_policy(nat.AW_STORE_NT):
            mid_hook()
    if dz_T is None:
        dz_T = _cast(dz, T)

    K.gemm(dz_T, sv.xR_T, D, H, N, a_trans=True, b_trans=True, C=slot(pr["sep"].weight).view(D, H), accumulate=True,
           a_rowsum=slot(pr["sep"].bias))
    gx, gxo = e(N, H, dt=RT), e(N, H, dt=T)
    K.gemm(dz_T, sv.Ws, N, H, D, b_trans=True, C=gx, C2=None if bnm else gxo, c2_mode=0 if bnm else
           (3 if R > 0 else 2), drop2=(p_drop, sv.enc.seeds[-1] if R > 0 else 0), seed_ptr=sv.ctr)

    gx, gxo, wgrads = resstack.backward(sv.enc, gx, gxo, sv.enc.ws, _grads(pr["enc"], slot), pr["enc_bn"], slot)
    K.wgrad_issue(wgrads)

    K.gemm(gxo, sv.patches, H, P, N, a_trans=True, b_trans=True, C=slot(pr["pe"].weight).view(H, P),
           accumulate=True, a_rowsum=slot(pr["pe"].bias))


class VQVAEPatchFunction(torch.autograd.Function):

    @staticmethod
    def forward(ctx, m, x, seed, *params):
        training = m.training
        need = torch.is_grad_enabled() or any(p.requires_grad for p in params)
        emb, x_hat, perp, idx, sv = forward(m, x, training, need_backward=True, seed=seed)
        ctx.m, ctx.sv, ctx.params = m, sv, params
        if perp is not None:
            ctx.mark_non_differentiable(perp)
        m._last_indices = idx
        return emb, x_hat, perp

    @staticmethod
    def backward(ctx, g_emb, g_xhat, g_perp):
        m, sv = ctx.m, ctx.sv
        sink = getattr(m, "_grad_sink", None)
        grads = {}

        def slot(p):
            if sink is not None and p in sink:
                return sink[p]
            g = grads.get(p)
            if g is None:
                g = torch.zeros_like(p, dtype=F32)
                grads[p] = g
            return g

        if g_emb is None:
            g_emb = torch.zeros(1, device=g_xhat.device)
        if g_xhat is None:
            g_xhat = torch.zeros(sv.sh.B, sv.sh.L, sv.sh.C, device=g_emb.device)
        backward(m, sv, g_emb.reshape(1).contiguous(), g_xhat, slot)
        ctx.sv = None
        return (None, None, None) + tuple(grads.get(p) for p in ctx.params)
```

### vq-vae-transformer-arc-welding_amd/csrc/reschain.hip

```cpp
#include "common.h"

#include <type_traits>

#pragma clang diagnostic ignored "-Winline-asm"


namespace {

constexpr int EC_H = 512;
constexpr int EC_ROWS = 64;
constexpr int EC_NTH = 512;
constexpr int EC_ROWB = EC_H * 2;
constexpr int EC_SCR = 2048;
constexpr int EC_SEG = 16;

template <int TAPS> struct EcGeo {
  static constexpr int KS = 16 * TAPS;
  static constexpr int JS = (TAPS == 1 ? 16 : 17) * EC_ROWB;
  static constexpr int R0 = TAPS == 1 ? 0 : EC_ROWB;
  static constexpr int IMG = (TAPS == 1 ? 64 : 69) * EC_ROWB;
  static constexpr int SCR = 2 * IMG;
  static constexpr int FLAGS = SCR + 8 * EC_SCR;
  static constexpr int BIAS = FLAGS + 64;
  static constexpr int LDS = BIAS + 8 * 256;
  static constexpr int TBIAS = LDS;
  static constexpr int LDS_TAIL = TBIAS + 8 * 256;
  static constexpr uint32_t WBYTES = (uint32_t)EC_H * EC_H * 2 * TAPS;
  static constexpr int WWAVE = 4 * KS * 1024;
  static constexpr uint64_t KEYS = TAPS == 1 ? 0xfe76dc54ba329810ull : 0xf53ac739685ace10ull;
  __device__ static int key(int u) { return u < 0 ? 15 : u > 15 ? 0 : (int)((KEYS >> (4 * u)) & 15); }
};
static_assert(EcGeo<3>::LDS_TAIL <= 160 * 1024, "decoder chain LDS");

typedef __amdgpu_buffer_rsrc_t rsrc_t;
__device__ __forceinline__ rsrc_t ec_rsrc(const void* p, uint32_t nbytes) {
  return __builtin_amdgcn_make_buffer_rsrc((void*)p, (short)0, p ? nbytes : 0u, 0x00020000);
}
__device__ __forceinline__ u32x2 ec_load8(rsrc_t r, uint32_t voff, int soff) {
  return __builtin_amdgcn_raw_buffer_load_b64(r, voff, soff, 0);
}
template <bool WT> __device__ __forceinline__ void ec_store16(rsrc_t r, uint32_t voff, int soff, uint4 v) {
  aw_v4i32 u;
  memcpy(&u, &v, 16);
  __builtin_amdgcn_raw_buffer_store_b128(u, r, voff, soff, WT ? 16 : 2);
  asm volatile("s_nop 1" ::"v"(u));
}
__device__ __forceinline__ void ec_store8(rsrc_t r, uint32_t voff, u32x2 v) {
  __builtin_amdgcn_raw_buffer_store_b64(v, r, voff, 0, 2);
}
typedef __attribute__((ext_vector_type(2))) __bf16 bf16x2;
__device__ __forceinline__ u32x2 ec_pack(const float (&v)[4]) {
  const bf16x2 lo = __builtin_convertvector((f32x2){v[0], v[1]}, bf16x2);
  const bf16x2 hi = __builtin_convertvector((f32x2){v[2], v[3]}, bf16x2);
  return u32x2{__builtin_bit_cast(uint32_t, lo), __builtin_bit_cast(uint32_t, hi)};
}
__device__ __forceinline__ void ec_unpack(u32x2 u, float (&v)[4]) {
  v[0] = __uint_as_float(u.x << 16);
  v[1] = __uint_as_float(u.x & 0xFFFF0000u);
  v[2] = __uint_as_float(u.y << 16);
  v[3] = __uint_as_float(u.y & 0xFFFF0000u);
}
__device__ __forceinline__ uint4 ec_wload(rsrc_t r, int voff, int soff) {
  const auto v = __builtin_amdgcn_raw_buffer_load_b128(r, voff, soff, 0);
  uint4 u;
  memcpy(&u, &v, 16);
  return u;
}
__device__ __forceinline__ void ec_lds_w8(char* smem, int off, u32x2 v) { *reinterpret_cast<u32x2*>(smem + off) = v; }
__device__ __forceinline__ uint4 ec_lds_r16(const char* smem, int off) {
  return *reinterpret_cast<const uint4*>(smem + off);
}

template <class G> __device__ __forceinline__ int ec_off(int tok, int chunk) {
  return G::R0 + (tok >> 4) * G::JS + (tok & 15) * EC_ROWB + ((chunk ^ G::key(tok & 15)) << 4);
}

template <class G>
__device__ __forceinline__ void ec_load_image(char* img, const void* src, int64_t row0, uint32_t nbytes, int tid) {
  const rsrc_t rs = ec_rsrc(src, nbytes);
#pragma unroll
  for (int q = 0; q < (EC_ROWS * EC_ROWB / 16) / EC_NTH; ++q) {
    const int c = tid + q * EC_NTH, tok = c >> 6, ch = c & 63;
    const uint32_t off = (uint32_t)((row0 + tok) * EC_ROWB + ch * 16);
    const auto v = __builtin_amdgcn_raw_buffer_load_b128(rs, off, 0, 0);
    uint4 u;
    memcpy(&u, &v, 16);
    *reinterpret_cast<uint4*>(img + ec_off<G>(tok, ch)) = u;
  }
  if constexpr (G::R0 != 0) {
    for (int c = tid; c < 2 * 5 * 64; c += EC_NTH) {
      const int im = c / 320, row = (c % 320) >> 6, ch = c & 63;
      *reinterpret_cast<uint4*>(img + im * G::IMG + row * G::JS + ch * 16) = uint4{0u, 0u, 0u, 0u};
    }
  }
}

typedef __attribute__((address_space(3))) volatile int lds_vint;
template <class G> __device__ __forceinline__ lds_vint* ec_flag(char* smem, int wv) {
  return (lds_vint*)(smem + G::FLAGS) + wv;
}
template <class G> __device__ __forceinline__ void ec_wait(char* smem, int wv, int target) {
  while (__builtin_amdgcn_readfirstlane(*ec_flag<G>(smem, wv)) < target) __builtin_amdgcn_s_sleep(1);
  asm volatile("" ::: "memory");
}
template <class G> __device__ __forceinline__ void ec_publish(char* smem, int w, int lane, int count) {
  asm volatile("s_waitcnt lgkmcnt(0)" ::: "memory");
  if (lane == 0) *ec_flag<G>(smem, w) = count;
}

__device__ __forceinline__ void ec_frag_fence(int) { __builtin_amdgcn_sched_barrier(0); }

__device__ __forceinline__ void ec_gelu_grad4(const float (&v)[4], float (&y)[4]) {
#pragma unroll
  for (int e = 0; e < 4; ++e) y[e] = gelu_erf_grad_fast(v[e]);
}
__device__ __forceinline__ void ec_gelu_and_grad4(const float (&v)[4], float (&y)[4], float (&d)[4]) {
#pragma unroll
  for (int e = 0; e < 4; ++e) {
    float ex;
    const float phi = aw_phi_e(v[e], ex);
    y[e] = v[e] * phi;
    d[e] = fmaf(v[e] * AW_INV_SQRT2PI, ex, phi);
  }
}

template <class G> __device__ __forceinline__ constexpr int ec_woff(int i, int s) { return (i * G::KS + s) * 1024; }

__device__ __forceinline__ size_t ec_keep_idx(int r, int tid) {
  return ((size_t)r * gridDim.x + blockIdx.x) * EC_NTH + tid;
}
__device__ __forceinline__ u32x2 ec_keep(const uint64_t* masks, int r, int tid) {
  return __builtin_bit_cast(u32x2, masks[ec_keep_idx(r, tid)]);
}
__device__ __forceinline__ uint32_t ec_keep_bits(uint64_t seed, uint64_t grp0, int f, uint32_t thr) {
  uint32_t lo = (uint32_t)grp0, hi = (uint32_t)(grp0 >> 32);
  asm volatile("" : "+v"(lo), "+v"(hi));
  const uint64_t h = aw_hash_group(seed, (((uint64_t)hi << 32) | lo) + 2048u * (f & 3) + 4u * (f >> 2));
  uint32_t k = 0;
#pragma unroll
  for (int e = 0; e < 4; ++e) k |= (((uint32_t)(h >> (16 * e)) & 0xFFFFu) >= thr ? 1u : 0u) << (4 * (f & 7) + e);
  return k;
}
__device__ __forceinline__ void ec_scales(u32x2 keep, int i, int j, float k, float (&ds)[4]) {
  const int f = 4 * i + j;
  const uint32_t b = ((f >> 3) ? keep.y : keep.x) >> (4 * (f & 7));
#pragma unroll
  for (int e = 0; e < 4; ++e) ds[e] = (b >> e) & 1u ? k : 0.f;
}

template <class G, int KS, bool MAYSKIP, typename Tail, typename Step>
__device__ __forceinline__ void ec_conv_g(f32x4 (&acc)[4][4], uint4 (&wf)[2][4], char* smem,
                                          const int (&rb)[G::KS / 16], int io, rsrc_t rc, rsrc_t rn, bool has_next,
                                          int wl, int wln, int nks, int w, int target, Tail tail, Step step) {
  constexpr int T = G::KS / 16, T0 = KS == G::KS ? 0 : T / 2;
  static_assert(KS == G::KS || KS == 16, "all taps or the centre tap");
#pragma unroll
  for (int i = 0; i < 4; ++i)
#pragma unroll
    for (int j = 0; j < 4; ++j) acc[i][j] = f32x4{0.f, 0.f, 0.f, 0.f};
  int rbi[T];
#pragma unroll
  for (int t = 0; t < T; ++t) rbi[t] = rb[t] + io;
#pragma unroll
  for (int s = 0; s < KS; ++s) {
    const int t = T0 + (s >> 4), kk = s & 15;
    if (s < 16 && (kk & 1) == 0 && (kk >> 1) != w && (!MAYSKIP || target >= 0)) ec_wait<G>(smem, kk >> 1, target);
    uint4 bf[4];
#pragma unroll
    for (int j = 0; j < 4; ++j) bf[j] = ec_lds_r16(smem, (rbi[t] ^ (64 * (kk & 3))) + (kk >> 2) * 256 + j * G::JS);
#pragma unroll
    for (int i = 0; i < 4; ++i)
#pragma unroll
      for (int j = 0; j < 4; ++j)
        acc[i][j] = __builtin_amdgcn_mfma_f32_16x16x32_bf16(__builtin_bit_cast(bf16x8, wf[s & 1][i]),
                                                            __builtin_bit_cast(bf16x8, bf[j]), acc[i][j], 0, 0, 0);
    if (s + 2 < KS) {
#pragma unroll
      for (int i = 0; i < 4; ++i) wf[s & 1][i] = ec_wload(rc, wl, (i * KS + s + 2) * 1024);
    } else if (has_next) {
#pragma unroll
      for (int i = 0; i < 4; ++i) wf[s & 1][i] = ec_wload(rn, wln, (i * nks + s + 2 - KS) * 1024);
    }
    step(s);
    if (s == KS - 1) tail();
    __builtin_amdgcn_sched_barrier(0);
  }
}
template <class G, typename Tail, typename Step>
__device__ __forceinline__ void ec_conv(f32x4 (&acc)[4][4], uint4 (&wf)[2][4], char* smem, const int (&rb)[G::KS / 16],
                                        int io, rsrc_t rc, rsrc_t rn, bool has_next, int wl, int w, int target,
                                        Tail tail, Step step) {
  constexpr int T = G::KS / 16;
#pragma unroll
  for (int i = 0; i < 4; ++i)
#pragma unroll
    for (int j = 0; j < 4; ++j) acc[i][j] = f32x4{0.f, 0.f, 0.f, 0.f};
  int rbi[T];
#pragma unroll
  for (int t = 0; t < T; ++t) rbi[t] = rb[t] + io;
#pragma unroll
  for (int s = 0; s < G::KS; ++s) {
    const int t = s >> 4, kk = s & 15;
    if (t == 0 && (kk & 1) == 0 && (kk >> 1) != w) ec_wait<G>(smem, kk >> 1, target);
    uint4 bf[4];
#pragma unroll
    for (int j = 0; j < 4; ++j) bf[j] = ec_lds_r16(smem, (rbi[t] ^ (64 * (kk & 3))) + (kk >> 2) * 256 + j * G::JS);
#pragma unroll
    for (int i = 0; i < 4; ++i)
#pragma unroll
      for (int j = 0; j < 4; ++j)
        acc[i][j] = __builtin_amdgcn_mfma_f32_16x16x32_bf16(__builtin_bit_cast(bf16x8, wf[s & 1][i]),
                                                            __builtin_bit_cast(bf16x8, bf[j]), acc[i][j], 0, 0, 0);
    if (s + 2 < G::KS) {
#pragma unroll
      for (int i = 0; i < 4; ++i) wf[s & 1][i] = ec_wload(rc, wl, ec_woff<G>(i, s + 2));
    } else if (has_next) {
#pragma unroll
      for (int i = 0; i < 4; ++i) wf[s & 1][i] = ec_wload(rn, wl, ec_woff<G>(i, s + 2 - G::KS));
    }
    step(s);
    if (s == G::KS - 1) tail();
    __builtin_amdgcn_sched_barrier(0);
  }
}

template <class G, int DIR> struct EcLane {
  static constexpr int T = G::KS / 16;
  int lane, li, g, w;
  int wl;
  int rb[T];
  int wb0;
  __device__ __forceinline__ EcLane(int tid) {
    lane = tid & 63;
    w = tid >> 6, g = lane >> 4, li = lane & 15;
    wl = w * G::WWAVE + lane * 16;
#pragma unroll
    for (int t = 0; t < T; ++t) {
      const int tp = li + (T == 1 ? 0 : DIR * (t - 1)), key = G::key(tp);
      rb[t] = G::R0 + tp * EC_ROWB + ((4 * (key >> 2) + (g ^ (key & 3))) << 4);
    }
    wb0 = G::R0 + li * EC_ROWB + (((8 * w + (g >> 1)) ^ G::key(li)) << 4) + (g & 1) * 8;
  }
  __device__ __forceinline__ int wb(int i) const { return wb0 ^ (32 * i); }
};
template <class G> struct EcStore {
  int ir[2];
  int sw[4];
  int sr;
  __device__ __forceinline__ int srq(int q) const { return q ? (sr ^ 64) + 1024 : sr; }
  uint32_t gs;
  __device__ __forceinline__ EcStore(int tid, int64_t row0) {
    const int lane = tid & 63, w = tid >> 6, g = lane >> 4, li = lane & 15;
    const int t8 = lane >> 3, c8 = lane & 7;
#pragma unroll
    for (int p = 0; p < 2; ++p) ir[p] = G::R0 + (8 * p + t8) * EC_ROWB + (((8 * w + c8) ^ G::key(8 * p + t8)) << 4);
    const int sbase = G::SCR + w * EC_SCR;
#pragma unroll
    for (int i = 0; i < 4; ++i) sw[i] = sbase + li * 128 + (((2 * i + (g >> 1)) ^ (li >> 1)) << 4) + (g & 1) * 8;
    sr = sbase + t8 * 128 + ((c8 ^ (t8 >> 1)) << 4);
    gs = (uint32_t)(((row0 + t8) * EC_H + 64 * w + 8 * c8) * 2);
  }
};

__device__ __forceinline__ void ec_load_frags(u32x2 (&d)[4][4], rsrc_t r, uint32_t go) {
#pragma unroll
  for (int i = 0; i < 4; ++i)
#pragma unroll
    for (int j = 0; j < 4; ++j) d[i][j] = ec_load8(r, go, 16384 * j + 32 * i);
}
__device__ __forceinline__ uint32_t ec_frag_off(int64_t row0, int li, int w, int g) {
  return (uint32_t)(((row0 + li) * EC_H + 64 * w + 4 * g) * 2);
}
template <class G, bool WT>
__device__ __forceinline__ void ec_store_slice(const char* smem, int img, const EcStore<G>& S, rsrc_t r) {
  const int b0 = img + S.ir[0], b1 = img + S.ir[1];
#pragma unroll
  for (int q = 0; q < 8; ++q)
    ec_store16<WT>(r, S.gs, 8192 * q, ec_lds_r16(smem, ((q & 1) ? b1 : b0) + G::JS * (q >> 1)));
}
template <class G, bool WT>
__device__ __forceinline__ void ec_store_scratch(const char* smem, int j, const EcStore<G>& S, rsrc_t r) {
#pragma unroll
  for (int q = 0; q < 2; ++q) ec_store16<WT>(r, S.gs, 8192 * (2 * j + q), ec_lds_r16(smem, S.srq(q)));
}

template <class G, bool WT>
__device__ __forceinline__ void ec_store_scratch_at(const char* smem, int j, const EcStore<G>& S, rsrc_t r,
                                                    uint32_t gs, int st8, int co) {
#pragma unroll
  for (int q = 0; q < 2; ++q) ec_store16<WT>(r, gs, st8 * (2 * j + q) + co, ec_lds_r16(smem, S.srq(q)));
}

template <class G> __device__ __forceinline__ void ec_init(char* smem, int tid) {
  if (tid < 8) *ec_flag<G>(smem, tid) = 0;
}

template <int TAPS, bool DROP, bool WT, bool TAIL>
__global__ __launch_bounds__(EC_NTH) void res_chain_fwd_kernel(aw_res_chain_fwd_args P) {
  using G = EcGeo<TAPS>;
  static_assert(!TAIL || TAPS == 3, "the ConvT tail follows the decoder chain");
  __shared__ __attribute__((aligned(16))) char smem[TAIL ? G::LDS_TAIL : G::LDS];
  const int tid = threadIdx.x;
  const int64_t row0 = (int64_t)blockIdx.x * EC_ROWS;
  const EcLane<G, 1> L(tid);
  const uint32_t nbytes = (uint32_t)(P.N * EC_ROWB);
  const int R = P.R, NC = 2 * R;

  ec_init<G>(smem, tid);
  if constexpr (TAIL) *reinterpret_cast<float*>(smem + G::TBIAS + 4 * tid) = P.tail_bias[tid];
  ec_load_image<G>(smem, P.a0, row0, nbytes, tid);
  u32x2 xr[4][4];
  ec_load_frags(xr, ec_rsrc(P.x0, nbytes), ec_frag_off(row0, L.li, L.w, L.g));
  uint4 wf[2][4];
  {
    const rsrc_t r0 = ec_rsrc(P.w1[0], G::WBYTES);
#pragma unroll
    for (int i = 0; i < 4; ++i) {
      wf[0][i] = ec_wload(r0, L.wl, ec_woff<G>(i, 0));
      wf[1][i] = ec_wload(r0, L.wl, ec_woff<G>(i, 1));
    }
  }
  const rsrc_t rmask = ec_rsrc(DROP ? P.drop_masks : nullptr, (uint32_t)(R * gridDim.x * EC_NTH * 8));
  const uint32_t thr = aw_drop_threshold(P.drop_p);
  const uint64_t grp0 = (uint64_t)(row0 + L.li) * (EC_H / 4) + 16 * L.w + L.g;
  asm volatile("s_waitcnt lgkmcnt(0)" ::: "memory");
  __syncthreads();

  for (int c = 0; c < NC; ++c) {
    const int r = c >> 1;
    const bool second = (c & 1) != 0;
    const rsrc_t rc = ec_rsrc(second ? P.w2[r] : P.w1[r], G::WBYTES);
    const bool tail_next = TAIL && c + 1 == NC;
    const bool has_next = TAIL || c + 1 < NC;
    const rsrc_t rn = ec_rsrc(tail_next ? P.tail_w[0] : has_next ? (second ? P.w1[r + 1] : P.w2[r]) : nullptr,
                              tail_next ? EcGeo<1>::WBYTES : G::WBYTES);
    const int io = (c & 1) * G::IMG, no = ((c + 1) & 1) * G::IMG;
    f32x4 acc[4][4];
    const float bias_l = (second ? P.b2[r] : P.b1[r])[64 * L.w + L.lane];
    const uint64_t seed = DROP && second ? aw_seed_mix(P.drop_seed[r], P.seed_ptr) : 0;
    uint32_t kb[2] = {0u, 0u};
    auto hash = [&](int s) {
      if (DROP && second && s < 16) kb[s >> 3] |= ec_keep_bits(seed, grp0, s, thr);
    };
    auto park = [&] {
      *reinterpret_cast<float*>(smem + G::BIAS + 256 * L.w + 4 * L.lane) = bias_l;
      if (DROP && second) ec_store8(rmask, (uint32_t)(ec_keep_idx(r, tid) * 8), u32x2{kb[0], kb[1]});
    };
    if constexpr (TAIL)
      ec_conv_g<G, G::KS, false>(acc, wf, smem, L.rb, io, rc, rn, true, L.wl,
                                 tail_next ? L.w * EcGeo<1>::WWAVE + L.lane * 16 : L.wl, tail_next ? 16 : G::KS, L.w, c,
                                 park, hash);
    else
      ec_conv<G>(acc, wf, smem, L.rb, io, rc, rn, has_next, L.wl, L.w, c, park, hash);
    const u32x2 keep = {kb[0], kb[1]};
    int nwb[4];
#pragma unroll
    for (int i = 0; i < 4; ++i) nwb[i] = L.wb(i) + no;

    auto bias = [&](int i, float (&bv)[4]) {
      const float4 b4 = *reinterpret_cast<const float4*>(smem + G::BIAS + 256 * L.w + 64 * i + 16 * L.g);
      bv[0] = b4.x, bv[1] = b4.y, bv[2] = b4.z, bv[3] = b4.w;
    };
    const EcStore<G> S(tid, row0);
    if (!second) {
      const rsrc_t rh = ec_rsrc(P.dgelu_h[r], nbytes);
#pragma unroll
      for (int j = 0; j < 4; ++j) {
#pragma unroll
        for (int i = 0; i < 4; ++i) {
          float v[4], y[4], d[4], bv[4];
          bias(i, bv);
#pragma unroll
          for (int e = 0; e < 4; ++e) v[e] = acc[i][j][e] + bv[e];
          ec_gelu_and_grad4(v, y, d);
          ec_lds_w8(smem, nwb[i] + G::JS * j, ec_pack(y));
          ec_lds_w8(smem, S.sw[i], ec_pack(d));
          ec_frag_fence(4 * j + i);
        }
        ec_store_scratch<G, WT>(smem, j, S, rh);
        __builtin_amdgcn_sched_barrier(0);
      }
      ec_publish<G>(smem, L.w, L.lane, c + 1);
      ec_store_slice<G, WT>(smem, no, S, ec_rsrc(P.a1[r], nbytes));
    } else {
      const bool last = r == R - 1;
      const float dk = DROP ? 1.f / (1.f - P.drop_p) : 1.f;
      auto resid = [&](int i, int j, float (&v)[4]) {
        float ds[4] = {1.f, 1.f, 1.f, 1.f}, xv[4], bv[4];
        bias(i, bv);
        if constexpr (DROP) ec_scales(keep, i, j, dk, ds);
        ec_unpack(xr[i][j], xv);
#pragma unroll
        for (int e = 0; e < 4; ++e) v[e] = aw_epi_mad(acc[i][j][e] + bv[e], ds[e], DROP, xv[e], true);
        xr[i][j] = ec_pack(v);
      };
      if (!last) {
        const rsrc_t rx = ec_rsrc(P.dgelu_x[r], nbytes);
#pragma unroll
        for (int j = 0; j < 4; ++j) {
#pragma unroll
          for (int i = 0; i < 4; ++i) {
            float v[4], y[4], d[4];
            resid(i, j, v);
            ec_gelu_and_grad4(v, y, d);
            ec_lds_w8(smem, nwb[i] + G::JS * j, ec_pack(y));
            ec_lds_w8(smem, S.sw[i], ec_pack(d));
            ec_frag_fence(4 * j + i);
          }
          ec_store_scratch<G, WT>(smem, j, S, rx);
          __builtin_amdgcn_sched_barrier(0);
        }
        ec_publish<G>(smem, L.w, L.lane, c + 1);
      } else {
#pragma unroll
        for (int i = 0; i < 4; ++i)
#pragma unroll
          for (int j = 0; j < 4; ++j) {
            float v[4];
            resid(i, j, v);
            ec_lds_w8(smem, nwb[i] + G::JS * j, xr[i][j]);
            ec_frag_fence(4 * i + j);
          }
        if constexpr (TAIL) ec_publish<G>(smem, L.w, L.lane, c + 1);
      }
      ec_store_slice<G, WT>(smem, no, S, ec_rsrc(P.a[r], nbytes));
    }
  }

  if constexpr (TAIL) {
    using G1 = EcGeo<1>;
    const int k1 = P.tail_k1;
    const int wl1 = L.w * G1::WWAVE + L.lane * 16;
    const EcStore<G> S(tid, row0);
    const rsrc_t ry = ec_rsrc(P.tail_y, (uint32_t)(P.N * k1 * EC_ROWB));
    const uint32_t ygs = (uint32_t)(((row0 + (L.lane >> 3)) * k1 * EC_H + 64 * L.w + 8 * (L.lane & 7)) * 2);
    const int st8 = 8 * k1 * EC_ROWB;
    const int64_t left = P.N - row0;
    const int ngrp = left >= EC_ROWS ? 4 : (int)(left >> 4);
    double cs[4][4], cq[4][4];
#pragma unroll
    for (int i = 0; i < 4; ++i)
#pragma unroll
      for (int e = 0; e < 4; ++e) cs[i][e] = cq[i][e] = 0.;
    for (int jt = 0; jt < k1; ++jt) {
      const bool more = jt + 1 < k1;
      const rsrc_t rc = ec_rsrc(P.tail_w[jt], G1::WBYTES);
      const rsrc_t rn = ec_rsrc(more ? P.tail_w[jt + 1] : nullptr, G1::WBYTES);
      f32x4 acc[4][4];
      ec_conv_g<G, 16, true>(acc, wf, smem, L.rb, 0, rc, rn, more, wl1, wl1, 16, L.w, jt == 0 ? NC : -1, [] {},
                             [](int) {});
#pragma unroll
      for (int j = 0; j < 4; ++j) {
        if (j < ngrp) {
#pragma unroll
          for (int i = 0; i < 4; ++i) {
            const float4 b4 = *reinterpret_cast<const float4*>(smem + G::TBIAS + 256 * L.w + 64 * i + 16 * L.g);
            const float bv[4] = {b4.x, b4.y, b4.z, b4.w};
            float v[4];
#pragma unroll
            for (int e = 0; e < 4; ++e) {
              v[e] = acc[i][j][e] + bv[e];
              const double vd = (double)v[e];
              cs[i][e] += vd;
              cq[i][e] += vd * vd;
            }
            ec_lds_w8(smem, S.sw[i], ec_pack(v));
            ec_frag_fence(4 * j + i);
          }
          ec_store_scratch_at<G, WT>(smem, j, S, ry, ygs, st8, jt * EC_ROWB);
        }
        __builtin_amdgcn_sched_barrier(0);
      }
    }
    if (P.tail_colstats) {
#pragma unroll
      for (int i = 0; i < 4; ++i)
#pragma unroll
        for (int e = 0; e < 4; ++e)
#pragma unroll
          for (int m = 1; m < 16; m <<= 1) {
            cs[i][e] += __shfl_xor(cs[i][e], m);
            cq[i][e] += __shfl_xor(cq[i][e], m);
          }
      double* red = reinterpret_cast<double*>(smem + G::SCR + L.w * EC_SCR);
      asm volatile("s_waitcnt lgkmcnt(0)" ::: "memory");
      if (L.li == 0) {
#pragma unroll
        for (int i = 0; i < 4; ++i)
#pragma unroll
          for (int e = 0; e < 4; ++e) {
            red[16 * i + 4 * L.g + e] = cs[i][e];
            red[64 + 16 * i + 4 * L.g + e] = cq[i][e];
          }
      }
      asm volatile("s_waitcnt lgkmcnt(0)" ::: "memory");
      const double a = red[L.lane], b = red[64 + L.lane];
      atomicAdd(P.tail_colstats + 64 * L.w + L.lane, a);
      atomicAdd(P.tail_colstats + EC_H + 64 * L.w + L.lane, b);
    }
  }
}

template <int TAPS, bool DROP, bool WT>
__global__ __launch_bounds__(EC_NTH) void res_chain_bwd_kernel(aw_res_chain_bwd_args P) {
  using G = EcGeo<TAPS>;
  __shared__ __attribute__((aligned(16))) char smem[G::LDS];
  const int tid = threadIdx.x;
  const int64_t row0 = (int64_t)blockIdx.x * EC_ROWS;
  const EcLane<G, -1> L(tid);
  const uint32_t nbytes = (uint32_t)(P.N * EC_ROWB);
  const int R = P.R, NC = 2 * R;
  const uint32_t fo = ec_frag_off(row0, L.li, L.w, L.g);

  ec_init<G>(smem, tid);
  ec_load_image<G>(smem, P.gxo, row0, nbytes, tid);
  u32x2 gr[4][4];
  ec_load_frags(gr, ec_rsrc(P.gx, nbytes), fo);
  uint4 wf[2][4];
  {
    const rsrc_t r0 = ec_rsrc(P.w2t[R - 1], G::WBYTES);
#pragma unroll
    for (int i = 0; i < 4; ++i) {
      wf[0][i] = ec_wload(r0, L.wl, ec_woff<G>(i, 0));
      wf[1][i] = ec_wload(r0, L.wl, ec_woff<G>(i, 1));
    }
  }
  asm volatile("s_waitcnt lgkmcnt(0)" ::: "memory");
  __syncthreads();

  for (int c = 0; c < NC; ++c) {
    const int r = R - 1 - (c >> 1);
    const bool second = (c & 1) != 0;
    const rsrc_t rc = ec_rsrc(second ? P.w1t[r] : P.w2t[r], G::WBYTES);
    const bool has_next = c + 1 < NC;
    const rsrc_t rn = ec_rsrc(has_next ? (second ? P.w2t[r - 1] : P.w1t[r]) : nullptr, G::WBYTES);
    const int io = (c & 1) * G::IMG, no = ((c + 1) & 1) * G::IMG;
    f32x4 acc[4][4];
    uint4 pl[8];
    u32x2 keep = {0u, 0u};
    auto load_pre = [&] {
      const rsrc_t rp = ec_rsrc(second ? (r > 0 ? P.dgelu_x[r] : P.x0) : P.dgelu_h[r], nbytes);
      const uint32_t gs = (uint32_t)(((row0 + (L.lane >> 3)) * EC_H + 64 * L.w + 8 * (L.lane & 7)) * 2);
#pragma unroll
      for (int q = 0; q < 8; ++q) {
        const auto v = __builtin_amdgcn_raw_buffer_load_b128(rp, gs, 8192 * q, 0);
        memcpy(&pl[q], &v, 16);
      }
      if (DROP && second && r > 0) keep = ec_keep(P.drop_masks, r - 1, tid);
    };
    ec_conv<G>(acc, wf, smem, L.rb, io, rc, rn, has_next, L.wl, L.w, c, load_pre, [](int) {});
    int nwb[4];
#pragma unroll
    for (int i = 0; i < 4; ++i) nwb[i] = L.wb(i) + no;
    const EcStore<G> S(tid, row0);
    auto stage_pre = [&](int j) {
      *reinterpret_cast<uint4*>(smem + S.srq(0)) = pl[2 * j];
      *reinterpret_cast<uint4*>(smem + S.srq(1)) = pl[2 * j + 1];
    };
    auto pre_frag = [&](int i, float (&pv)[4]) { ec_unpack(*reinterpret_cast<const u32x2*>(smem + S.sw[i]), pv); };

    if (!second) {
#pragma unroll
      for (int j = 0; j < 4; ++j) {
        stage_pre(j);
#pragma unroll
        for (int i = 0; i < 4; ++i) {
          float ag[4], v[4];
          pre_frag(i, ag);
#pragma unroll
          for (int e = 0; e < 4; ++e) v[e] = aw_epi_mad(acc[i][j][e], ag[e], true, 0.f, false);
          ec_lds_w8(smem, nwb[i] + G::JS * j, ec_pack(v));
          ec_frag_fence(4 * j + i);
        }
      }
      ec_publish<G>(smem, L.w, L.lane, c + 1);
      ec_store_slice<G, WT>(smem, no, S, ec_rsrc(P.gh[r], nbytes));
    } else {
      auto grad = [&](int i, int j, float (&v)[4], auto raw) {
        float pv[4], gv[4], ag[4];
        pre_frag(i, pv);
        ec_unpack(gr[i][j], gv);
        if constexpr (decltype(raw)::value) {
          ec_gelu_grad4(pv, ag);
        } else {
#pragma unroll
          for (int e = 0; e < 4; ++e) ag[e] = pv[e];
        }
#pragma unroll
        for (int e = 0; e < 4; ++e) v[e] = aw_epi_mad(acc[i][j][e], ag[e], true, gv[e], true);
        gr[i][j] = ec_pack(v);
      };
      if (r > 0) {
        const float dk = DROP ? 1.f / (1.f - P.drop_p) : 1.f;
#pragma unroll
        for (int j = 0; j < 4; ++j) {
          stage_pre(j);
#pragma unroll
          for (int i = 0; i < 4; ++i) {
            float v[4], ds[4] = {1.f, 1.f, 1.f, 1.f}, o[4];
            grad(i, j, v, std::false_type{});
            if constexpr (DROP) ec_scales(keep, i, j, dk, ds);
#pragma unroll
            for (int e = 0; e < 4; ++e) o[e] = v[e] * ds[e];
            ec_lds_w8(smem, nwb[i] + G::JS * j, ec_pack(o));
            ec_frag_fence(4 * j + i);
          }
        }
        ec_publish<G>(smem, L.w, L.lane, c + 1);
      } else {
#pragma unroll
        for (int j = 0; j < 4; ++j) {
          stage_pre(j);
#pragma unroll
          for (int i = 0; i < 4; ++i) {
            float v[4];
            grad(i, j, v, std::true_type{});
            ec_lds_w8(smem, nwb[i] + G::JS * j, gr[i][j]);
            ec_frag_fence(4 * j + i);
          }
        }
      }
      ec_store_slice<G, WT>(smem, no, S, ec_rsrc(P.gxo_out[r], nbytes));
    }
  }
}

struct PackJobs {
  const void* src[AW_RES_PACK_MAX];
  void* fwd[AW_RES_PACK_MAX];
  void* bwd[AW_RES_PACK_MAX];
  uint32_t one_tap;
};

constexpr int PK_PITCH1 = 128 + 16;
template <int TAPS>
__device__ __forceinline__ void res_pack_fwd(const char* __restrict__ W, uint4* __restrict__ out, char* t, int x,
                                             int nx, int tid) {
  constexpr int RB = EC_ROWB * TAPS, PITCH0 = RB + 16, KB = 16 * TAPS;
  for (int mb = x; mb < EC_H / 16; mb += nx) {
#pragma unroll
    for (int q = 0; q < 4 * TAPS; ++q) {
      const int c = tid + 256 * q, row = c / (64 * TAPS), kc = c % (64 * TAPS);
      *reinterpret_cast<uint4*>(t + row * PITCH0 + kc * 16) =
          *reinterpret_cast<const uint4*>(W + (size_t)(16 * mb + row) * RB + kc * 16);
    }
    __syncthreads();
#pragma unroll
    for (int q = 0; q < 4 * TAPS; ++q) {
      const int o = tid + 256 * q, st = o >> 6, l = o & 63;
      out[(size_t)mb * 64 * KB + o] = *reinterpret_cast<const uint4*>(t + (l & 15) * PITCH0 + (4 * st + (l >> 4)) * 16);
    }
    __syncthreads();
  }
}
template <int TAPS>
__global__ __launch_bounds__(256) void res_pack_kernel(PackJobs J) {
  constexpr int RB = EC_ROWB * TAPS, PITCH0 = RB + 16, KB = 16 * TAPS;
  constexpr int SZ = 16 * PITCH0 > EC_H * PK_PITCH1 ? 16 * PITCH0 : EC_H * PK_PITCH1;
  __shared__ __attribute__((aligned(16))) char t[SZ];
  const int x = blockIdx.x, job = blockIdx.y, tid = threadIdx.x;
  const char* __restrict__ W = reinterpret_cast<const char*>(J.src[job]);
  const bool one_tap = TAPS > 1 && ((J.one_tap >> job) & 1u);
  if (blockIdx.z == 0) {
    uint4* __restrict__ out = reinterpret_cast<uint4*>(J.fwd[job]);
    if (!out) return;
    if (one_tap) res_pack_fwd<1>(W, out, t, x, (int)gridDim.x, tid);
    else res_pack_fwd<TAPS>(W, out, t, x, (int)gridDim.x, tid);
  } else {
    uint4* __restrict__ out = reinterpret_cast<uint4*>(J.bwd[job]);
    if (!out || one_tap) return;
    const int tap = x >> 3, b = x & 7;
#pragma unroll
    for (int q = 0; q < 16; ++q) {
      const int c = tid + 256 * q, o = c >> 3, kc = c & 7;
      *reinterpret_cast<uint4*>(t + o * PK_PITCH1 + kc * 16) =
          *reinterpret_cast<const uint4*>(W + (size_t)o * RB + tap * EC_ROWB + 128 * b + kc * 16);
    }
    __syncthreads();
#pragma unroll 4
    for (int q = 0; q < 16; ++q) {
      const int o = tid + 256 * q, mb = o >> 10, st = (o >> 6) & 15, l = o & 63, li = l & 15, g = l >> 4;
      uint16_t e[8];
#pragma unroll
      for (int k = 0; k < 8; ++k)
        e[k] = *reinterpret_cast<const uint16_t*>(t + (32 * st + 8 * g + k) * PK_PITCH1 + (16 * mb + li) * 2);
      uint4 v;
      memcpy(&v, e, 16);
      out[((size_t)(4 * b + mb) * KB + 16 * tap + st) * 64 + l] = v;
    }
  }
}

struct MaskSeeds {
  uint64_t seed[AW_RES_CHAIN_MAX];
};
__global__ __launch_bounds__(EC_NTH) void res_mask_kernel(MaskSeeds S, const uint64_t* seed_ptr, uint32_t thr,
                                                          u32x2* __restrict__ out) {
  const int tid = threadIdx.x, r = blockIdx.y;
  const int lane = tid & 63, w = tid >> 6, g = lane >> 4, li = lane & 15;
  const uint64_t seed = aw_seed_mix(S.seed[r], seed_ptr);
  const uint64_t grp0 = (((uint64_t)blockIdx.x * EC_ROWS + li) * EC_H >> 2) + 16 * w + g;
  uint32_t k[2] = {0u, 0u};
#pragma unroll
  for (int f = 0; f < 16; ++f) k[f >> 3] |= ec_keep_bits(seed, grp0, f, thr);
  out[((size_t)r * gridDim.x + blockIdx.x) * EC_NTH + tid] = u32x2{k[0], k[1]};
}

bool aligned16(const void* p) { return ((uintptr_t)p & 15) == 0; }

template <int TAPS, bool TAIL>
void launch_fwd(const aw_res_chain_fwd_args* a, bool drop, bool wt, dim3 grid, hipStream_t s) {
  if (drop && wt) hipLaunchKernelGGL((res_chain_fwd_kernel<TAPS, true, true, TAIL>), grid, dim3(EC_NTH), 0, s, *a);
  else if (drop) hipLaunchKernelGGL((res_chain_fwd_kernel<TAPS, true, false, TAIL>), grid, dim3(EC_NTH), 0, s, *a);
  else if (wt) hipLaunchKernelGGL((res_chain_fwd_kernel<TAPS, false, true, TAIL>), grid, dim3(EC_NTH), 0, s, *a);
  else hipLaunchKernelGGL((res_chain_fwd_kernel<TAPS, false, false, TAIL>), grid, dim3(EC_NTH), 0, s, *a);
}
template <int TAPS>
void launch_bwd(const aw_res_chain_bwd_args* a, bool drop, bool wt, dim3 grid, hipStream_t s) {
  if (drop && wt) hipLaunchKernelGGL((res_chain_bwd_kernel<TAPS, true, true>), grid, dim3(EC_NTH), 0, s, *a);
  else if (drop) hipLaunchKernelGGL((res_chain_bwd_kernel<TAPS, true, false>), grid, dim3(EC_NTH), 0, s, *a);
  else if (wt) hipLaunchKernelGGL((res_chain_bwd_kernel<TAPS, false, true>), grid, dim3(EC_NTH), 0, s, *a);
  else hipLaunchKernelGGL((res_chain_bwd_kernel<TAPS, false, false>), grid, dim3(EC_NTH), 0, s, *a);
}

}

#define CHAIN_SHAPE_CHECKS(who)                                                                                       \
  AW_REQUIRE(a, who ": null args");                                                                                   \
  AW_REQUIRE(a->H == EC_H, who ": H must be %d (got %d)", EC_H, a->H);                                                \
  AW_REQUIRE(a->R >= 1 && a->R <= AW_RES_CHAIN_MAX, who ": R must be 1..%d", AW_RES_CHAIN_MAX);                       \
  AW_REQUIRE(a->N >= 1 && (a->N + EC_ROWS) * EC_ROWB < (1ll << 31), who ": N out of range");                          \
  AW_REQUIRE(a->taps == 1 || (a->taps == 3 && a->seg == EC_SEG && a->N % EC_SEG == 0),                                \
             who ": taps must be 1, or 3 with seg == %d and N %% %d == 0 (taps %d, seg %d)", EC_SEG, EC_SEG, a->taps, \
             a->seg);                                                                                                 \
  AW_REQUIRE(a->drop_p >= 0.f && a->drop_p < 1.f, who ": drop_p out of [0, 1)")

extern "C" int aw_res_chain_fwd(const aw_res_chain_fwd_args* a, void* stream) {
  CHAIN_SHAPE_CHECKS("aw_res_chain_fwd");
  AW_REQUIRE(a->a0 && a->x0 && aligned16(a->a0) && aligned16(a->x0), "aw_res_chain_fwd: a0 / x0 missing or unaligned");
  for (int r = 0; r < a->R; ++r) {
    AW_REQUIRE(a->w1[r] && a->w2[r] && a->b1[r] && a->b2[r] && aligned16(a->w1[r]) && aligned16(a->w2[r]) &&
               aligned16(a->b1[r]) && aligned16(a->b2[r]), "aw_res_chain_fwd: block %d weights missing or unaligned", r);
    AW_REQUIRE(a->a[r] && aligned16(a->a[r]), "aw_res_chain_fwd: block %d output a missing or unaligned", r);
    AW_REQUIRE(aligned16(a->dgelu_h[r]) && aligned16(a->a1[r]) && aligned16(a->dgelu_x[r]),
               "aw_res_chain_fwd: block %d saved outputs unaligned", r);
  }
  AW_REQUIRE(aligned16(a->drop_masks), "aw_res_chain_fwd: drop_masks unaligned");
  if (a->tail_k1 == 0) {
    AW_REQUIRE(!a->tail_bias && !a->tail_y && !a->tail_colstats, "aw_res_chain_fwd: tail fields without tail_k1");
  } else {
    AW_REQUIRE(a->taps == 3 && a->tail_k1 >= 1 && a->tail_k1 <= AW_RES_TAIL_MAX,
               "aw_res_chain_fwd: the tail needs taps == 3 and tail_k1 in 1..%d (got %d)", AW_RES_TAIL_MAX, a->tail_k1);
    AW_REQUIRE((a->N + EC_ROWS) * a->tail_k1 * EC_ROWB < (1ll << 31), "aw_res_chain_fwd: N * tail_k1 out of range");
    AW_REQUIRE(a->tail_y && aligned16(a->tail_y) && a->tail_bias && ((uintptr_t)a->tail_colstats & 7) == 0,
               "aw_res_chain_fwd: tail_y / tail_bias missing or unaligned");
    for (int j = 0; j < a->tail_k1; ++j)
      AW_REQUIRE(a->tail_w[j] && aligned16(a->tail_w[j]), "aw_res_chain_fwd: tail matrix %d missing or unaligned", j);
  }
  hipStream_t s = (hipStream_t)stream;
  const dim3 grid((unsigned)((a->N + EC_ROWS - 1) / EC_ROWS));
  const bool drop = a->drop_p > 0.f, wt = a->store_policy == AW_STORE_WT;
  if (a->tail_k1) launch_fwd<3, true>(a, drop, wt, grid, s);
  else if (a->taps == 3) launch_fwd<3, false>(a, drop, wt, grid, s);
  else launch_fwd<1, false>(a, drop, wt, grid, s);
  return aw::check_launch("aw_res_chain_fwd");
}

extern "C" int aw_res_chain_bwd(const aw_res_chain_bwd_args* a, void* stream) {
  CHAIN_SHAPE_CHECKS("aw_res_chain_bwd");
  AW_REQUIRE(a->gx && a->gxo && a->x0 && aligned16(a->gx) && aligned16(a->gxo) && aligned16(a->x0),
             "aw_res_chain_bwd: gx / gxo / x0 missing or unaligned");
  for (int r = 0; r < a->R; ++r) {
    AW_REQUIRE(a->w1t[r] && a->w2t[r] && aligned16(a->w1t[r]) && aligned16(a->w2t[r]),
               "aw_res_chain_bwd: block %d weights missing or unaligned", r);
    AW_REQUIRE(a->dgelu_h[r] && aligned16(a->dgelu_h[r]) && (r == 0 || (a->dgelu_x[r] && aligned16(a->dgelu_x[r]))),
               "aw_res_chain_bwd: block %d saved GELU' missing or unaligned", r);
    AW_REQUIRE(a->gh[r] && a->gxo_out[r] && aligned16(a->gh[r]) && aligned16(a->gxo_out[r]),
               "aw_res_chain_bwd: block %d outputs missing or unaligned", r);
  }
  AW_REQUIRE(a->drop_p == 0.f || a->R == 1 || (a->drop_masks && aligned16(a->drop_masks)),
             "aw_res_chain_bwd: drop_p > 0 needs drop_masks");
  hipStream_t s = (hipStream_t)stream;
  const dim3 grid((unsigned)((a->N + EC_ROWS - 1) / EC_ROWS));
  const bool drop = a->drop_p > 0.f && a->R > 1, wt = a->store_policy == AW_STORE_WT;
  if (a->taps == 3) launch_bwd<3>(a, drop, wt, grid, s);
  else launch_bwd<1>(a, drop, wt, grid, s);
  return aw::check_launch("aw_res_chain_bwd");
}

extern "C" int aw_res_pack_weights(const void* const* src, void* const* fwd, void* const* bwd, int n, int taps,
                                   void* stream) {
  return aw_res_pack_weights_mixed(src, fwd, bwd, nullptr, n, taps, stream);
}

extern "C" int aw_res_pack_weights_mixed(const void* const* src, void* const* fwd, void* const* bwd,
                                         const int* job_taps, int n, int taps, void* stream) {
  AW_REQUIRE(src && fwd && bwd && n >= 0 && n <= AW_RES_PACK_MAX && (taps == 1 || taps == 3),
             "aw_res_pack_weights: bad args (n must be 0..%d, taps 1 or 3)", AW_RES_PACK_MAX);
  if (n == 0) return AW_OK;
  PackJobs J{};
  for (int i = 0; i < n; ++i) {
    AW_REQUIRE(src[i] && aligned16(src[i]) && aligned16(fwd[i]) && aligned16(bwd[i]) && (fwd[i] || bwd[i]) &&
                   src[i] != fwd[i] && src[i] != bwd[i], "aw_res_pack_weights: job %d: missing, aliased or unaligned", i);
    J.src[i] = src[i];
    J.fwd[i] = fwd[i];
    J.bwd[i] = bwd[i];
    if (job_taps && job_taps[i] != taps) {
      AW_REQUIRE(job_taps[i] == 1 && fwd[i] && !bwd[i], "aw_res_pack_weights: job %d: a job of %d taps in a launch of "
                 "%d (only 1-tap forward copies may differ)", i, job_taps[i], taps);
      J.one_tap |= 1u << i;
    }
  }
  const dim3 grid(8 * taps, n, 2);
  if (taps == 3) hipLaunchKernelGGL(res_pack_kernel<3>, grid, dim3(256), 0, (hipStream_t)stream, J);
  else hipLaunchKernelGGL(res_pack_kernel<1>, grid, dim3(256), 0, (hipStream_t)stream, J);
  return aw::check_launch("aw_res_pack_weights");
}

extern "C" int64_t aw_res_dropout_masks_bytes(int64_t N, int R) {
  if (N < 1 || R < 1 || R > AW_RES_CHAIN_MAX) return -1;
  return (int64_t)R * ((N + EC_ROWS - 1) / EC_ROWS) * EC_NTH * 8;
}

extern "C" int aw_res_dropout_masks(int64_t N, int R, float drop_p, const uint64_t* drop_seed, const uint64_t* seed_ptr,
                                    void* masks, void* stream) {
  AW_REQUIRE(N >= 1 && R >= 1 && R <= AW_RES_CHAIN_MAX && drop_seed && masks && aligned16(masks) && drop_p > 0.f &&
                 drop_p < 1.f, "aw_res_dropout_masks: bad args");
  MaskSeeds S{};
  for (int r = 0; r < R; ++r) S.seed[r] = drop_seed[r];
  hipLaunchKernelGGL(res_mask_kernel, dim3((unsigned)((N + EC_ROWS - 1) / EC_ROWS), R), dim3(EC_NTH), 0,
                     (hipStream_t)stream, S, seed_ptr, aw_drop_threshold(drop_p), (u32x2*)masks);
  return aw::check_launch("aw_res_dropout_masks");
}
```

Before: 433,800 windows/s.

## Fuse input-gradient head GEMM into residual chain backward kernel

The standalone GEMMs that turned the upstream gradient (gY2·Wt1 in the decoder, dz·Ws in the encoder) into gx/gxo before the residual-chain backward are replaced by a head stage inside res_chain_bwd_kernel. That stage loads the head gradient and packed head weights, accumulates them into the chain's LDS image, and applies dropout. The head weights are packed in the same launch as the chain weights, using new BWD1/K64 pack modes. This removes a separate kernel launch and the round trip of two NxH gradient tensors through HBM, at the cost of more kernel template variants and extra prologue work per block.

Result: no change. 436,800 windows/s, median of 6 (+0.7%).

```diff
diff --git a/include/arcweld_amd.h b/include/arcweld_amd.h
--- a/include/arcweld_amd.h
+++ b/include/arcweld_amd.h
@@ -98,6 +98,12 @@
   float drop_p;
   int store_policy;
   const uint64_t* drop_masks;
+  int head_n;
+  int head_ks;
+  const void* head_w[AW_RES_TAIL_MAX];
+  const void* head_g;
+  int64_t head_ld;
+  void* head_gxo;
 } aw_res_chain_bwd_args;
 int aw_res_chain_fwd(const aw_res_chain_fwd_args* args, void* stream);
 int aw_res_chain_bwd(const aw_res_chain_bwd_args* args, void* stream);
@@ -106,6 +112,8 @@
                          void* masks, void* stream);
 #define AW_RES_PACK_MAX 32
 int aw_res_pack_weights(const void* const* src, void* const* fwd, void* const* bwd, int n, int taps, void* stream);
+#define AW_RES_PACK_BWD1 (-1)
+#define AW_RES_PACK_K64 (-64)
 int aw_res_pack_weights_mixed(const void* const* src, void* const* fwd, void* const* bwd, const int* job_taps, int n,
                               int taps, void* stream);
 
diff --git a/vq-vae-transformer-arc-welding_amd/arcweld/_native.py b/vq-vae-transformer-arc-welding_amd/arcweld/_native.py
--- a/vq-vae-transformer-arc-welding_amd/arcweld/_native.py
+++ b/vq-vae-transformer-arc-welding_amd/arcweld/_native.py
@@ -61,6 +61,8 @@
 RES_CHAIN_MAX = 16
 RES_PACK_MAX = 32
 RES_TAIL_MAX = 8
+RES_PACK_BWD1 = -1
+RES_PACK_K64 = -64
 _E = RES_CHAIN_MAX
 
 
@@ -78,7 +80,9 @@
     _fields_ = [("N", c_i64), ("H", c_int), ("R", c_int), ("taps", c_int), ("seg", c_int), ("gx", c_p), ("gxo", c_p),
                 ("x0", c_p), ("w1t", c_p * _E), ("w2t", c_p * _E), ("dgelu_h", c_p * _E), ("dgelu_x", c_p * _E),
                 ("gh", c_p * _E), ("gxo_out", c_p * _E),
-                ("drop_p", c_f), ("store_policy", c_int), ("drop_masks", c_p)]
+                ("drop_p", c_f), ("store_policy", c_int), ("drop_masks", c_p),
+                ("head_n", c_int), ("head_ks", c_int), ("head_w", c_p * RES_TAIL_MAX), ("head_g", c_p),
+                ("head_ld", c_i64), ("head_gxo", c_p)]
 
 SIGNATURES = {
     "aw_version": [],
diff --git a/vq-vae-transformer-arc-welding_amd/arcweld/kernels.py b/vq-vae-transformer-arc-welding_amd/arcweld/kernels.py
--- a/vq-vae-transformer-arc-welding_amd/arcweld/kernels.py
+++ b/vq-vae-transformer-arc-welding_amd/arcweld/kernels.py
@@ -258,6 +258,11 @@
     return os.environ.get("ARCWELD_CONVT_TAIL", "1") != "0"
 
 
+def bwd_head_ok():
+    import os
+    return os.environ.get("ARCWELD_BWD_HEAD", "1") != "0"
+
+
 def res_chain_fwd(a0, x0, w1, w2, b1, b2, dh, a1, dx, a, drop=(0.0, None), seed_ptr=None, masks=None, taps=1, seg=16,
                   stream=None, tail=None):
     N, H = a0.shape
@@ -304,11 +309,14 @@
                                   list(dx)[:-1] + list(a) + extra)))
 
 
-def res_chain_bwd(gx, gxo, w1t, w2t, dh, x0, dx, gh, gxo_out, drop_p=0.0, masks=None, taps=1, seg=16, stream=None):
-    N, H = gx.shape
+def res_chain_bwd(gx, gxo, w1t, w2t, dh, x0, dx, gh, gxo_out, drop_p=0.0, masks=None, taps=1, seg=16, stream=None,
+                  head=None):
+    N, H = x0.shape
     R = len(w1t)
     if not (1 <= R <= RES_CHAIN_MAX) or not all(len(v) == R for v in (w2t, dh, dx, gh, gxo_out)):
         raise nat.NativeError("res_chain_bwd: need R (1..16) entries in every per-block list")
+    if (head is None) == (gx is None) or (gx is None) != (gxo is None):
+        raise nat.NativeError("res_chain_bwd: pass either gx and gxo, or a head")
     _chk_rows([gx, gxo, x0] + list(dh) + list(dx[1:]) + list(gh) + list(gxo_out), N, H, "res_chain_bwd")
     g = nat.ResChainBwdArgs()
     g.N, g.H, g.R, g.taps, g.seg = N, H, R, int(taps), int(seg)
@@ -320,11 +328,29 @@
     g.drop_p = float(drop_p)
     g.store_policy = _chain_store_policy()
     g.drop_masks = ptr(masks)
-    _maybe_timed(stream, "gemm_bf16", _chain_flops(R, N, H, taps, seg),
+    flops, extra = _chain_flops(R, N, H, taps, seg), []
+    if head is not None:
+        hg, wh, hgxo = head
+        hk = 16 if taps == 3 else 2
+        if hg.dtype != torch.bfloat16 or hg.dim() != 2 or hg.shape[0] != N or not hg.is_contiguous():
+            raise nat.NativeError(f"res_chain_bwd: head g must be a contiguous ({N}, ld) bfloat16 tensor")
+        if not (1 <= len(wh) <= nat.RES_TAIL_MAX) or hg.shape[1] != len(wh) * 32 * hk:
+            raise nat.NativeError(f"res_chain_bwd: head g needs {32 * hk} columns per matrix, 1..{nat.RES_TAIL_MAX} "
+                                  "matrices")
+        for w in wh:
+            if w.dtype != torch.bfloat16 or w.numel() != H * 32 * hk or not w.is_contiguous():
+                raise nat.NativeError(f"res_chain_bwd: head matrices must be packed ({H}, {32 * hk}) bfloat16 copies")
+        _chk_rows([hgxo], N, H, "res_chain_bwd")
+        g.head_n, g.head_ks, g.head_g, g.head_ld, g.head_gxo = len(wh), hk, ptr(hg), hg.shape[1], ptr(hgxo)
+        for j, w in enumerate(wh):
+            g.head_w[j] = ptr(w)
+        flops += 2.0 * N * hg.shape[1] * H
+        extra = [hg, hgxo] + list(wh)
+    _maybe_timed(stream, "gemm_bf16", flops,
                  lambda sp: call("aw_res_chain_bwd", ctypes.byref(g), sp),
                  lambda: (f"res_chain_bwd_kernel<{int(taps)}>",
                           _nbytes([gx, gxo, x0, masks] + list(w1t) + list(w2t) + list(dh) + list(dx[1:]) + list(gh) +
-                                  list(gxo_out))))
+                                  list(gxo_out) + extra)))
 
 
 def res_pack_weights(src, fwd=None, bwd=None, taps=1, stream=None, job_taps=None):
@@ -336,8 +362,9 @@
         raise nat.NativeError("res_pack_weights: list lengths differ")
     for i in range(n):
         for t in (src[i], fwd[i], bwd[i]):
-            if t is not None and (t.dtype != torch.bfloat16 or t.numel() != 512 * 512 * jt[i] or not t.is_contiguous()):
-                raise nat.NativeError(f"res_pack_weights: need contiguous 512 x {512 * jt[i]} bfloat16 tensors")
+            k = 64 if jt[i] == nat.RES_PACK_K64 else 512 if jt[i] == nat.RES_PACK_BWD1 else 512 * jt[i]
+            if t is not None and (t.dtype != torch.bfloat16 or t.numel() != 512 * k or not t.is_contiguous()):
+                raise nat.NativeError(f"res_pack_weights: need contiguous 512 x {k} bfloat16 tensors")
     for c0 in range(0, n, nat.RES_PACK_MAX):
         sl = slice(c0, c0 + nat.RES_PACK_MAX)
         m = len(src[sl])
diff --git a/vq-vae-transformer-arc-welding_amd/arcweld/resstack.py b/vq-vae-transformer-arc-welding_amd/arcweld/resstack.py
--- a/vq-vae-transformer-arc-welding_amd/arcweld/resstack.py
+++ b/vq-vae-transformer-arc-welding_amd/arcweld/resstack.py
@@ -156,23 +156,36 @@
         K.res_pack_weights(wsrc, pk, None, taps=taps)
     if save:
         sv.pk_bwd = wsrc
-        if sv.p_drop > 0 and R > 1:
+        if sv.p_drop > 0 and R > 0:
             sv.masks = K.res_dropout_masks_empty(N, R, dev)
     K.res_chain_fwd(a0, x0, pk[0::2], pk[1::2], [b1 for b1, _ in biases], [b2 for _, b2 in biases], sv.hs, sv.a1s,
                     sv.xs[1:], sv.a0s[1:], drop=(sv.p_drop, sv.seeds), seed_ptr=sv.ctr, masks=sv.masks, taps=taps,
                     seg=geo.S, tail=ktail)
 
 
-def _chain_bwd(sv, gx, gxo, grads):
-    N, H = gx.shape
+def _chain_bwd(sv, gx, gxo, grads, head=None):
     geo = sv.geo
-    R, taps, dev, T = len(sv.hs), geo.taps, gx.device, gxo.dtype
+    N, H = sv.xs[0].shape
+    R, taps, dev, T = len(sv.hs), geo.taps, sv.xs[0].device, sv.T
     gh = [torch.empty(N, H, device=dev, dtype=T) for _ in range(R)]
     go = [torch.empty(N, H, device=dev, dtype=T) for _ in range(R)]
     pk_bwd = [torch.empty(H, geo.Kd, device=dev, dtype=T) for _ in sv.pk_bwd]
-    K.res_pack_weights(sv.pk_bwd, None, pk_bwd, taps=taps)
-    K.res_chain_bwd(gx, gxo, pk_bwd[0::2], pk_bwd[1::2], sv.hs, sv.xs[0], [None] + list(sv.xs[1:R]), gh, go,
-                    drop_p=sv.p_drop, masks=sv.masks, taps=taps, seg=geo.S)
+    khead = None
+    if head is not None:
+        g, W = head
+        if taps == 3:
+            hsrc, jt = [W[j * H:(j + 1) * H] for j in range(W.shape[0] // H)], K.nat.RES_PACK_BWD1
+        else:
+            hsrc, jt = [W], K.nat.RES_PACK_K64
+        hpk = [torch.empty(H, w.shape[0], device=dev, dtype=T) for w in hsrc]
+        K.res_pack_weights(list(sv.pk_bwd) + hsrc, None, pk_bwd + hpk, taps=taps,
+                           job_taps=[taps] * len(pk_bwd) + [jt] * len(hsrc))
+        gxo = torch.empty(N, H, device=dev, dtype=T)
+        khead = (g, hpk, gxo)
+    else:
+        K.res_pack_weights(sv.pk_bwd, None, pk_bwd, taps=taps)
+    K.res_chain_bwd(gx, None if khead else gxo, pk_bwd[0::2], pk_bwd[1::2], sv.hs, sv.xs[0], [None] + list(sv.xs[1:R]),
+                    gh, go, drop_p=sv.p_drop, masks=sv.masks, taps=taps, seg=geo.S, head=khead)
     sv.pk_bwd = sv.masks = None
     wgrads = []
     for r in reversed(range(R)):
@@ -221,9 +234,11 @@
     return x, a, sv
 
 
-def backward(sv, gy, go, dweights, grads, bns=None, slot=None, r0_copy=True):
+def backward(sv, gy, go, dweights, grads, bns=None, slot=None, r0_copy=True, head=None):
+    if head is not None and (sv.route != "chain" or gy is not None or go is not None):
+        raise ValueError("resstack.backward: the input-gradient head runs only inside a chain, in place of gy / go")
     if sv.route == "chain":
-        gxo, wgrads = _chain_bwd(sv, gy, go, grads)
+        gxo, wgrads = _chain_bwd(sv, gy, go, grads, head)
         return gxo, gxo, wgrads
     N, H = gy.shape
     geo, RT, T, p = sv.geo, gy.dtype, sv.T, sv.p_drop
diff --git a/vq-vae-transformer-arc-welding_amd/arcweld/vqvae.py b/vq-vae-transformer-arc-welding_amd/arcweld/vqvae.py
--- a/vq-vae-transformer-arc-welding_amd/arcweld/vqvae.py
+++ b/vq-vae-transformer-arc-welding_amd/arcweld/vqvae.py
@@ -313,13 +313,18 @@
     K.gemm(sv.yR_T, gY2, H, k1 * H, N, a_trans=True, b_trans=True, C=slot(pr["t1"].weight).view(H, H * k1),
            accumulate=True, col_map=(H, k1, 0))
     RT = sv.RT
-    gy, go = e(N, H, dt=RT), e(N, H, dt=T)
     bnm = m.batch_norm and R > 0
-    K.gemm(gY2, sv.Wt1, N, H, k1 * H, b_trans=True, C=gy, C2=None if bnm else go, c2_mode=0 if bnm else
-           (3 if R > 0 else 2), drop2=(p_drop, sv.dec.seeds[-1] if R > 0 else 0), seed_ptr=sv.ctr)
+    heads = K.bwd_head_ok() and T == torch.bfloat16
+    dec_head = heads and sv.dec.route == "chain" and k1 <= nat.RES_TAIL_MAX
+    gy = go = None
+    if not dec_head:
+        gy, go = e(N, H, dt=RT), e(N, H, dt=T)
+        K.gemm(gY2, sv.Wt1, N, H, k1 * H, b_trans=True, C=gy, C2=None if bnm else go, c2_mode=0 if bnm else
+               (3 if R > 0 else 2), drop2=(p_drop, sv.dec.seeds[-1] if R > 0 else 0), seed_ptr=sv.ctr)
 
     dgw = [(sv.ops[f"dgw{r}_1"], sv.ops[f"dgw{r}_2"]) for r in range(R)]
-    gy, go, wgrads = resstack.backward(sv.dec, gy, go, dgw, _grads(pr["dec"], slot), pr["dec_bn"], slot)
+    gy, go, wgrads = resstack.backward(sv.dec, gy, go, dgw, _grads(pr["dec"], slot), pr["dec_bn"], slot,
+                                       head=(gY2, sv.Wt1) if dec_head else None)
     K.gemm_grouped(wgrads)
 
     K.gemm(go, sv.zq_T, H, D, N, a_trans=True, b_trans=True, C=slot(pr["dec0"].weight).view(H, D), accumulate=True,
@@ -345,11 +350,15 @@
 
     K.gemm(dz_T, sv.xR_T, D, H, N, a_trans=True, b_trans=True, C=slot(pr["sep"].weight).view(D, H), accumulate=True,
            a_rowsum=slot(pr["sep"].bias))
-    gx, gxo = e(N, H, dt=RT), e(N, H, dt=T)
-    K.gemm(dz_T, sv.Ws, N, H, D, b_trans=True, C=gx, C2=None if bnm else gxo, c2_mode=0 if bnm else
-           (3 if R > 0 else 2), drop2=(p_drop, sv.enc.seeds[-1] if R > 0 else 0), seed_ptr=sv.ctr)
-
-    gx, gxo, wgrads = resstack.backward(sv.enc, gx, gxo, sv.enc.ws, _grads(pr["enc"], slot), pr["enc_bn"], slot)
+    enc_head = heads and sv.enc.route == "chain" and D == 64
+    gx = gxo = None
+    if not enc_head:
+        gx, gxo = e(N, H, dt=RT), e(N, H, dt=T)
+        K.gemm(dz_T, sv.Ws, N, H, D, b_trans=True, C=gx, C2=None if bnm else gxo, c2_mode=0 if bnm else
+               (3 if R > 0 else 2), drop2=(p_drop, sv.enc.seeds[-1] if R > 0 else 0), seed_ptr=sv.ctr)
+
+    gx, gxo, wgrads = resstack.backward(sv.enc, gx, gxo, sv.enc.ws, _grads(pr["enc"], slot), pr["enc_bn"], slot,
+                                        head=(dz_T, sv.Ws) if enc_head else None)
     K.wgrad_issue(wgrads)
 
     K.gemm(gxo, sv.patches, H, P, N, a_trans=True, b_trans=True, C=slot(pr["pe"].weight).view(H, P),
diff --git a/vq-vae-transformer-arc-welding_amd/csrc/reschain.hip b/vq-vae-transformer-arc-welding_amd/csrc/reschain.hip
--- a/vq-vae-transformer-arc-welding_amd/csrc/reschain.hip
+++ b/vq-vae-transformer-arc-welding_amd/csrc/reschain.hip
@@ -148,16 +148,18 @@
   for (int e = 0; e < 4; ++e) ds[e] = (b >> e) & 1u ? k : 0.f;
 }
 
-template <class G, int KS, bool MAYSKIP, typename Tail, typename Step>
+template <class G, int KS, bool MAYSKIP, bool KEEP, typename Tail, typename Step>
 __device__ __forceinline__ void ec_conv_g(f32x4 (&acc)[4][4], uint4 (&wf)[2][4], char* smem,
                                           const int (&rb)[G::KS / 16], int io, rsrc_t rc, rsrc_t rn, bool has_next,
                                           int wl, int wln, int nks, int w, int target, Tail tail, Step step) {
   constexpr int T = G::KS / 16, T0 = KS == G::KS ? 0 : T / 2;
-  static_assert(KS == G::KS || KS == 16, "all taps or the centre tap");
-#pragma unroll
-  for (int i = 0; i < 4; ++i)
-#pragma unroll
-    for (int j = 0; j < 4; ++j) acc[i][j] = f32x4{0.f, 0.f, 0.f, 0.f};
+  static_assert(KS == G::KS || KS == 16 || KS == 2, "all taps, the centre tap or its first 64 channels");
+  if constexpr (!KEEP) {
+#pragma unroll
+    for (int i = 0; i < 4; ++i)
+#pragma unroll
+      for (int j = 0; j < 4; ++j) acc[i][j] = f32x4{0.f, 0.f, 0.f, 0.f};
+  }
   int rbi[T];
 #pragma unroll
   for (int t = 0; t < T; ++t) rbi[t] = rb[t] + io;
@@ -347,7 +349,7 @@
       if (DROP && second) ec_store8(rmask, (uint32_t)(ec_keep_idx(r, tid) * 8), u32x2{kb[0], kb[1]});
     };
     if constexpr (TAIL)
-      ec_conv_g<G, G::KS, false>(acc, wf, smem, L.rb, io, rc, rn, true, L.wl,
+      ec_conv_g<G, G::KS, false, false>(acc, wf, smem, L.rb, io, rc, rn, true, L.wl,
                                  tail_next ? L.w * EcGeo<1>::WWAVE + L.lane * 16 : L.wl, tail_next ? 16 : G::KS, L.w, c,
                                  park, hash);
     else
@@ -447,7 +449,7 @@
       const rsrc_t rc = ec_rsrc(P.tail_w[jt], G1::WBYTES);
       const rsrc_t rn = ec_rsrc(more ? P.tail_w[jt + 1] : nullptr, G1::WBYTES);
       f32x4 acc[4][4];
-      ec_conv_g<G, 16, true>(acc, wf, smem, L.rb, 0, rc, rn, more, wl1, wl1, 16, L.w, jt == 0 ? NC : -1, [] {},
+      ec_conv_g<G, 16, true, false>(acc, wf, smem, L.rb, 0, rc, rn, more, wl1, wl1, 16, L.w, jt == 0 ? NC : -1, [] {},
                              [](int) {});
 #pragma unroll
       for (int j = 0; j < 4; ++j) {
@@ -501,7 +503,7 @@
   }
 }
 
-template <int TAPS, bool DROP, bool WT>
+template <int TAPS, bool DROP, bool WT, bool HEAD>
 __global__ __launch_bounds__(EC_NTH) void res_chain_bwd_kernel(aw_res_chain_bwd_args P) {
   using G = EcGeo<TAPS>;
   __shared__ __attribute__((aligned(16))) char smem[G::LDS];
@@ -511,22 +513,113 @@
   const uint32_t nbytes = (uint32_t)(P.N * EC_ROWB);
   const int R = P.R, NC = 2 * R;
   const uint32_t fo = ec_frag_off(row0, L.li, L.w, L.g);
+  const int hb = HEAD ? P.head_n : 0;
 
   ec_init<G>(smem, tid);
-  ec_load_image<G>(smem, P.gxo, row0, nbytes, tid);
   u32x2 gr[4][4];
-  ec_load_frags(gr, ec_rsrc(P.gx, nbytes), fo);
   uint4 wf[2][4];
-  {
-    const rsrc_t r0 = ec_rsrc(P.w2t[R - 1], G::WBYTES);
-#pragma unroll
-    for (int i = 0; i < 4; ++i) {
-      wf[0][i] = ec_wload(r0, L.wl, ec_woff<G>(i, 0));
-      wf[1][i] = ec_wload(r0, L.wl, ec_woff<G>(i, 1));
-    }
-  }
-  asm volatile("s_waitcnt lgkmcnt(0)" ::: "memory");
-  __syncthreads();
+  if constexpr (HEAD) {
+    constexpr int HKS = TAPS == 3 ? 16 : 2;
+    constexpr uint32_t HBYTES = (uint32_t)EC_H * 32 * HKS * 2;
+    const int hn = hb;
+    const int wlh = L.w * (4 * HKS * 1024) + L.lane * 16;
+    const rsrc_t rg = ec_rsrc(P.head_g, (uint32_t)(P.N * P.head_ld * 2));
+    const uint32_t st8 = (uint32_t)(8 * P.head_ld * 2);
+    const uint32_t hgs = (uint32_t)(((row0 + (L.lane >> 3)) * P.head_ld + 64 * L.w + 8 * (L.lane & 7)) * 2);
+    const bool mine = TAPS == 3 || L.w == 0;
+    uint4 pl[8];
+    auto load_g = [&](int j) {
+      if (mine) {
+#pragma unroll
+        for (int q = 0; q < 8; ++q) {
+          const auto v = __builtin_amdgcn_raw_buffer_load_b128(rg, hgs + (uint32_t)j * (64 * HKS) + st8 * q, 0, 0);
+          memcpy(&pl[q], &v, 16);
+        }
+      }
+    };
+    auto put_g = [&](int img) {
+      const EcStore<G> S(tid, row0);
+      if (mine) {
+#pragma unroll
+        for (int q = 0; q < 8; ++q)
+          *reinterpret_cast<uint4*>(smem + img + S.ir[q & 1] + G::JS * (q >> 1)) = pl[q];
+      }
+    };
+    load_g(0);
+    {
+      const rsrc_t r0 = ec_rsrc(P.head_w[0], HBYTES);
+#pragma unroll
+      for (int i = 0; i < 4; ++i) {
+        wf[0][i] = ec_wload(r0, wlh, (i * HKS) * 1024);
+        wf[1][i] = ec_wload(r0, wlh, (i * HKS + 1) * 1024);
+      }
+    }
+    if constexpr (G::R0 != 0) {
+      for (int c = tid; c < 2 * 5 * 64; c += EC_NTH) {
+        const int im = c / 320, row = (c % 320) >> 6, ch = c & 63;
+        *reinterpret_cast<uint4*>(smem + im * G::IMG + row * G::JS + ch * 16) = uint4{0u, 0u, 0u, 0u};
+      }
+    }
+    put_g((hn & 1) * G::IMG);
+    asm volatile("s_waitcnt lgkmcnt(0)" ::: "memory");
+    __syncthreads();
+
+    f32x4 acc[4][4];
+#pragma unroll
+    for (int i = 0; i < 4; ++i)
+#pragma unroll
+      for (int j = 0; j < 4; ++j) acc[i][j] = f32x4{0.f, 0.f, 0.f, 0.f};
+    u32x2 keep = {0u, 0u};
+    auto head_conv = [&](int j, auto last) {
+      constexpr bool LAST = decltype(last)::value;
+      const rsrc_t rc = ec_rsrc(P.head_w[j], HBYTES);
+      const rsrc_t rn = ec_rsrc(LAST ? P.w2t[R - 1] : P.head_w[j + 1], LAST ? G::WBYTES : HBYTES);
+      const int io = ((hn - j) & 1) * G::IMG, no = ((hn - j + 1) & 1) * G::IMG;
+      auto next = [&] {
+        if constexpr (!LAST) load_g(j + 1);
+        else if (DROP) keep = ec_keep(P.drop_masks, R - 1, tid);
+      };
+      ec_conv_g<G, HKS, false, true>(acc, wf, smem, L.rb, io, rc, rn, true, wlh, LAST ? L.wl : wlh,
+                                     LAST ? G::KS : HKS, L.w, j, next, [](int) {});
+      if constexpr (!LAST) {
+        put_g(no);
+        ec_publish<G>(smem, L.w, L.lane, j + 1);
+      }
+    };
+    for (int j = 0; j + 1 < hn; ++j) head_conv(j, std::false_type{});
+    head_conv(hn - 1, std::true_type{});
+    const EcStore<G> S(tid, row0);
+    const float dk = DROP ? 1.f / (1.f - P.drop_p) : 1.f;
+#pragma unroll
+    for (int j = 0; j < 4; ++j)
+#pragma unroll
+      for (int i = 0; i < 4; ++i) {
+        float v[4], ds[4] = {1.f, 1.f, 1.f, 1.f}, o[4];
+#pragma unroll
+        for (int e = 0; e < 4; ++e) v[e] = acc[i][j][e];
+        gr[i][j] = ec_pack(v);
+        if constexpr (DROP) ec_scales(keep, i, j, dk, ds);
+#pragma unroll
+        for (int e = 0; e < 4; ++e) o[e] = v[e] * ds[e];
+        ec_lds_w8(smem, L.wb(i) + G::JS * j, DROP ? ec_pack(o) : gr[i][j]);
+        ec_frag_fence(4 * j + i);
+      }
+    ec_publish<G>(smem, L.w, L.lane, hn);
+    ec_store_slice<G, WT>(smem, 0, S, ec_rsrc(P.head_gxo, nbytes));
+  } else {
+    ec_load_image<G>(smem, P.gxo, row0, nbytes, tid);
+    ec_load_frags(gr, ec_rsrc(P.gx, nbytes), fo);
+    {
+      const rsrc_t r0 = ec_rsrc(P.w2t[R - 1], G::WBYTES);
+#pragma unroll
+      for (int i = 0; i < 4; ++i) {
+        wf[0][i] = ec_wload(r0, L.wl, ec_woff<G>(i, 0));
+        wf[1][i] = ec_wload(r0, L.wl, ec_woff<G>(i, 1));
+      }
+    }
+    asm volatile("s_waitcnt lgkmcnt(0)" ::: "memory");
+    __syncthreads();
+  }
 
   for (int c = 0; c < NC; ++c) {
     const int r = R - 1 - (c >> 1);
@@ -548,7 +641,7 @@
       }
       if (DROP && second && r > 0) keep = ec_keep(P.drop_masks, r - 1, tid);
     };
-    ec_conv<G>(acc, wf, smem, L.rb, io, rc, rn, has_next, L.wl, L.w, c, load_pre, [](int) {});
+    ec_conv<G>(acc, wf, smem, L.rb, io, rc, rn, has_next, L.wl, L.w, hb + c, load_pre, [](int) {});
     int nwb[4];
 #pragma unroll
     for (int i = 0; i < 4; ++i) nwb[i] = L.wb(i) + no;
@@ -573,7 +666,7 @@
           ec_frag_fence(4 * j + i);
         }
       }
-      ec_publish<G>(smem, L.w, L.lane, c + 1);
+      ec_publish<G>(smem, L.w, L.lane, hb + c + 1);
       ec_store_slice<G, WT>(smem, no, S, ec_rsrc(P.gh[r], nbytes));
     } else {
       auto grad = [&](int i, int j, float (&v)[4], auto raw) {
@@ -606,7 +699,7 @@
             ec_frag_fence(4 * j + i);
           }
         }
-        ec_publish<G>(smem, L.w, L.lane, c + 1);
+        ec_publish<G>(smem, L.w, L.lane, hb + c + 1);
       } else {
 #pragma unroll
         for (int j = 0; j < 4; ++j) {
@@ -630,6 +723,7 @@
   void* fwd[AW_RES_PACK_MAX];
   void* bwd[AW_RES_PACK_MAX];
   uint32_t one_tap;
+  uint32_t k64;
 };
 
 constexpr int PK_PITCH1 = 128 + 16;
@@ -661,20 +755,43 @@
   const int x = blockIdx.x, job = blockIdx.y, tid = threadIdx.x;
   const char* __restrict__ W = reinterpret_cast<const char*>(J.src[job]);
   const bool one_tap = TAPS > 1 && ((J.one_tap >> job) & 1u);
+  const bool k64 = (J.k64 >> job) & 1u;
   if (blockIdx.z == 0) {
     uint4* __restrict__ out = reinterpret_cast<uint4*>(J.fwd[job]);
-    if (!out) return;
+    if (!out || k64) return;
     if (one_tap) res_pack_fwd<1>(W, out, t, x, (int)gridDim.x, tid);
     else res_pack_fwd<TAPS>(W, out, t, x, (int)gridDim.x, tid);
   } else {
     uint4* __restrict__ out = reinterpret_cast<uint4*>(J.bwd[job]);
-    if (!out || one_tap) return;
+    if (!out || (one_tap && x >= 8)) return;
     const int tap = x >> 3, b = x & 7;
+    const int rbj = one_tap ? EC_ROWB : RB, kbj = one_tap ? 16 : KB;
+    if (k64) {
+#pragma unroll
+      for (int q = 0; q < 2; ++q) {
+        const int c = tid + 256 * q, o = c >> 3, kc = c & 7;
+        *reinterpret_cast<uint4*>(t + o * PK_PITCH1 + kc * 16) =
+            *reinterpret_cast<const uint4*>(W + (size_t)o * EC_ROWB + 128 * b + kc * 16);
+      }
+      __syncthreads();
+#pragma unroll
+      for (int q = 0; q < 2; ++q) {
+        const int o = tid + 256 * q, mb = o >> 7, st = (o >> 6) & 1, l = o & 63, li = l & 15, g = l >> 4;
+        uint16_t e[8];
+#pragma unroll
+        for (int k = 0; k < 8; ++k)
+          e[k] = *reinterpret_cast<const uint16_t*>(t + (32 * st + 8 * g + k) * PK_PITCH1 + (16 * mb + li) * 2);
+        uint4 v;
+        memcpy(&v, e, 16);
+        out[((size_t)(4 * b + mb) * 2 + st) * 64 + l] = v;
+      }
+      return;
+    }
 #pragma unroll
     for (int q = 0; q < 16; ++q) {
       const int c = tid + 256 * q, o = c >> 3, kc = c & 7;
       *reinterpret_cast<uint4*>(t + o * PK_PITCH1 + kc * 16) =
-          *reinterpret_cast<const uint4*>(W + (size_t)o * RB + tap * EC_ROWB + 128 * b + kc * 16);
+          *reinterpret_cast<const uint4*>(W + (size_t)o * rbj + tap * EC_ROWB + 128 * b + kc * 16);
     }
     __syncthreads();
 #pragma unroll 4
@@ -686,7 +803,7 @@
         e[k] = *reinterpret_cast<const uint16_t*>(t + (32 * st + 8 * g + k) * PK_PITCH1 + (16 * mb + li) * 2);
       uint4 v;
       memcpy(&v, e, 16);
-      out[((size_t)(4 * b + mb) * KB + 16 * tap + st) * 64 + l] = v;
+      out[((size_t)(4 * b + mb) * kbj + 16 * tap + st) * 64 + l] = v;
     }
   }
 }
@@ -715,12 +832,12 @@
   else if (wt) hipLaunchKernelGGL((res_chain_fwd_kernel<TAPS, false, true, TAIL>), grid, dim3(EC_NTH), 0, s, *a);
   else hipLaunchKernelGGL((res_chain_fwd_kernel<TAPS, false, false, TAIL>), grid, dim3(EC_NTH), 0, s, *a);
 }
-template <int TAPS>
+template <int TAPS, bool HEAD>
 void launch_bwd(const aw_res_chain_bwd_args* a, bool drop, bool wt, dim3 grid, hipStream_t s) {
-  if (drop && wt) hipLaunchKernelGGL((res_chain_bwd_kernel<TAPS, true, true>), grid, dim3(EC_NTH), 0, s, *a);
-  else if (drop) hipLaunchKernelGGL((res_chain_bwd_kernel<TAPS, true, false>), grid, dim3(EC_NTH), 0, s, *a);
-  else if (wt) hipLaunchKernelGGL((res_chain_bwd_kernel<TAPS, false, true>), grid, dim3(EC_NTH), 0, s, *a);
-  else hipLaunchKernelGGL((res_chain_bwd_kernel<TAPS, false, false>), grid, dim3(EC_NTH), 0, s, *a);
+  if (drop && wt) hipLaunchKernelGGL((res_chain_bwd_kernel<TAPS, true, true, HEAD>), grid, dim3(EC_NTH), 0, s, *a);
+  else if (drop) hipLaunchKernelGGL((res_chain_bwd_kernel<TAPS, true, false, HEAD>), grid, dim3(EC_NTH), 0, s, *a);
+  else if (wt) hipLaunchKernelGGL((res_chain_bwd_kernel<TAPS, false, true, HEAD>), grid, dim3(EC_NTH), 0, s, *a);
+  else hipLaunchKernelGGL((res_chain_bwd_kernel<TAPS, false, false, HEAD>), grid, dim3(EC_NTH), 0, s, *a);
 }
 
 }
@@ -768,8 +885,25 @@
 
 extern "C" int aw_res_chain_bwd(const aw_res_chain_bwd_args* a, void* stream) {
   CHAIN_SHAPE_CHECKS("aw_res_chain_bwd");
-  AW_REQUIRE(a->gx && a->gxo && a->x0 && aligned16(a->gx) && aligned16(a->gxo) && aligned16(a->x0),
-             "aw_res_chain_bwd: gx / gxo / x0 missing or unaligned");
+  AW_REQUIRE(a->x0 && aligned16(a->x0), "aw_res_chain_bwd: x0 missing or unaligned");
+  if (a->head_n == 0) {
+    AW_REQUIRE(!a->head_ks && !a->head_g && !a->head_ld && !a->head_gxo,
+               "aw_res_chain_bwd: head fields without head_n");
+    AW_REQUIRE(a->gx && a->gxo && aligned16(a->gx) && aligned16(a->gxo),
+               "aw_res_chain_bwd: gx / gxo missing or unaligned");
+  } else {
+    const int ks = a->taps == 3 ? 16 : 2;
+    AW_REQUIRE(!a->gx && !a->gxo, "aw_res_chain_bwd: a head makes gx / gxo itself: both must be NULL");
+    AW_REQUIRE(a->head_n >= 1 && a->head_n <= AW_RES_TAIL_MAX && a->head_ks == ks && (ks == 16 || a->head_n == 1),
+               "aw_res_chain_bwd: the head needs head_n in 1..%d of head_ks = 16 (taps 3), or one of head_ks = 2 "
+               "(taps 1) (got head_n %d, head_ks %d)", AW_RES_TAIL_MAX, a->head_n, a->head_ks);
+    AW_REQUIRE(a->head_ld >= (int64_t)a->head_n * ks * 32 && a->head_ld % 8 == 0 &&
+                   (a->N + EC_ROWS) * a->head_ld * 2 < (1ll << 31), "aw_res_chain_bwd: head_ld out of range");
+    AW_REQUIRE(a->head_g && aligned16(a->head_g) && a->head_gxo && aligned16(a->head_gxo),
+               "aw_res_chain_bwd: head_g / head_gxo missing or unaligned");
+    for (int j = 0; j < a->head_n; ++j)
+      AW_REQUIRE(a->head_w[j] && aligned16(a->head_w[j]), "aw_res_chain_bwd: head matrix %d missing or unaligned", j);
+  }
   for (int r = 0; r < a->R; ++r) {
     AW_REQUIRE(a->w1t[r] && a->w2t[r] && aligned16(a->w1t[r]) && aligned16(a->w2t[r]),
                "aw_res_chain_bwd: block %d weights missing or unaligned", r);
@@ -778,13 +912,16 @@
     AW_REQUIRE(a->gh[r] && a->gxo_out[r] && aligned16(a->gh[r]) && aligned16(a->gxo_out[r]),
                "aw_res_chain_bwd: block %d outputs missing or unaligned", r);
   }
-  AW_REQUIRE(a->drop_p == 0.f || a->R == 1 || (a->drop_masks && aligned16(a->drop_masks)),
+  AW_REQUIRE(a->drop_p == 0.f || (a->R == 1 && !a->head_n) || (a->drop_masks && aligned16(a->drop_masks)),
              "aw_res_chain_bwd: drop_p > 0 needs drop_masks");
   hipStream_t s = (hipStream_t)stream;
   const dim3 grid((unsigned)((a->N + EC_ROWS - 1) / EC_ROWS));
-  const bool drop = a->drop_p > 0.f && a->R > 1, wt = a->store_policy == AW_STORE_WT;
-  if (a->taps == 3) launch_bwd<3>(a, drop, wt, grid, s);
-  else launch_bwd<1>(a, drop, wt, grid, s);
+  const bool drop = a->drop_p > 0.f && (a->R > 1 || a->head_n), wt = a->store_policy == AW_STORE_WT;
+  if (a->head_n) {
+    if (a->taps == 3) launch_bwd<3, true>(a, drop, wt, grid, s);
+    else launch_bwd<1, true>(a, drop, wt, grid, s);
+  } else if (a->taps == 3) launch_bwd<3, false>(a, drop, wt, grid, s);
+  else launch_bwd<1, false>(a, drop, wt, grid, s);
   return aw::check_launch("aw_res_chain_bwd");
 }
 
@@ -806,9 +943,13 @@
     J.fwd[i] = fwd[i];
     J.bwd[i] = bwd[i];
     if (job_taps && job_taps[i] != taps) {
-      AW_REQUIRE(job_taps[i] == 1 && fwd[i] && !bwd[i], "aw_res_pack_weights: job %d: a job of %d taps in a launch of "
-                 "%d (only 1-tap forward copies may differ)", i, job_taps[i], taps);
-      J.one_tap |= 1u << i;
+      AW_REQUIRE((job_taps[i] == 1 && fwd[i] && !bwd[i]) || (job_taps[i] == AW_RES_PACK_BWD1 && !fwd[i]) ||
+                     (job_taps[i] == AW_RES_PACK_K64 && taps == 1 && !fwd[i]),
+                 "aw_res_pack_weights: job %d: a job of %d taps in a launch of %d (only 1-tap forward copies, "
+                 "AW_RES_PACK_BWD1 backward copies, and AW_RES_PACK_K64 ones in a 1-tap launch, may differ)", i,
+                 job_taps[i], taps);
+      if (job_taps[i] == AW_RES_PACK_K64) J.k64 |= 1u << i;
+      else J.one_tap |= 1u << i;
     }
   }
   const dim3 grid(8 * taps, n, 2);
```
